# giuliop/AlgoPlonk

Hardware: AMD Instinct MI355X
Metric: proofs/sec (higher is better)
Workload: dtype u32x8 (Montgomery Fr/Fp)

## Files before the change

### algoplonk_amd/_lib.py

```python
from __future__ import annotations

import ctypes as C
import os

_HERE = os.path.dirname(os.path.abspath(__file__))
LIB_PATH = os.environ.get("APK_LIB") or os.path.join(_HERE, "libapk.so")

APK_BN254 = 0
APK_BLS12_381 = 1
APK_OK = 0
APK_ERR_ARG, APK_ERR_HIP, APK_ERR_STATE, APK_ERR_WITNESS, APK_ERR_VERIFY = 1, 2, 3, 4, 5
ABI_VERSION = 5
G1_MAX = 96
G2_MAX = 192
MAX_COMMITMENTS = 2
NB_BLINDING = 9

SYMBOLS = [
    "apk_last_error", "apk_abi_version", "apk_device_count", "apk_g1_bytes", "apk_fp_bytes",
    "apk_ctx_create", "apk_ctx_destroy", "apk_msm_ctx_create", "apk_ctx_get_vk", "apk_msm_g1", "apk_msm_g1_device", "apk_msm_g1_batch_device", "apk_ctx_set_commit_hook", "apk_device_copy", "apk_ntt",
    "apk_prove", "apk_prove_device", "apk_verify", "apk_verify_ex", "apk_g2_decompress", "apk_g2_mul_generator", "apk_g1_mul_batch", "apk_g1_decompress", "apk_g1_to_lagrange", "apk_marshal_proof", "apk_marshal_public_inputs",
    "apk_fe_from_be", "apk_fe_to_be", "apk_hash_fr", "apk_host_fe_op", "apk_host_g1_op", "apk_g1_sum",
    "apk_device_fe_op", "apk_device_g1_op", "apk_host_feu_op", "apk_device_feu_op", "apk_feu_shape", "apk_device_poly_op",
    "apk_device_alloc", "apk_device_free", "apk_device_upload", "apk_device_download",
    "apk_host_alloc", "apk_host_free", "apk_host_register", "apk_host_unregister",
    "apk_stats_enable", "apk_stats_read", "apk_paths_read",
    "apk_ctx_set_wire_hook", "apk_coset_ntt_device",
    "apk_comm_create", "apk_comm_destroy", "apk_comm_rank", "apk_comm_world", "apk_comm_barrier", "apk_comm_max_f64", "apk_comm_bind",
    "apk_comm_transport", "apk_msm_g1_sharded", "apk_comm_split_begin", "apk_comm_split_end", "apk_comm_serve", "apk_comm_set_compute",
    "apk_comm_commit", "apk_comm_wires", "apk_comm_rccl_ranks", "apk_comm_rccl_selftest",
    "apk_comm_commit_local", "apk_comm_spmd_begin", "apk_comm_spmd_end", "apk_comm_allgather_device", "apk_comm_subcoset_active",
    "apk_ctx_set_subcoset", "apk_comm_transport_reason", "apk_comm_link_probe", "apk_comm_phase_ms", "apk_ctx_msm_window",
    "apk_verify_batch", "apk_g1_lincomb_segments", "apk_device_sched_read", "apk_runtime_read",
    "apk_kzg_open", "apk_kzg_open_device", "apk_kzg_batch_open", "apk_kzg_batch_open_device", "apk_kzg_verify", "apk_kzg_batch_verify",
    "apk_kzg_fold_challenge", "apk_kzg_shape",
    "apk_kzg_open_lagrange", "apk_kzg_open_lagrange_device", "apk_kzg_batch_open_lagrange", "apk_kzg_batch_open_lagrange_device",
    "apk_kzg_lagrange_shape",
    "apk_kzg_open_multi", "apk_kzg_open_multi_device", "apk_kzg_batch_verify_multi", "apk_kzg_multi_weights",
    "apk_kzg_open_multi_lagrange", "apk_kzg_open_multi_lagrange_device",
    "apk_kzg_all_prepare", "apk_kzg_open_all", "apk_kzg_open_all_device",
    "apk_kzg_cosets_prepare", "apk_kzg_open_cosets", "apk_kzg_open_cosets_device", "apk_kzg_verify_coset",
    "apk_kzg_batch_verify_cosets", "apk_kzg_cosets_weights", "apk_kzg_cosets_fold", "apk_kzg_cosets_phase_ms",
    "apk_proof_blob_len", "apk_unmarshal_proof", "apk_unmarshal_public_inputs", "apk_verify_blob", "apk_verify_batch_keys", "apk_verify_blobs",
]


class ApkError(RuntimeError):
    def __init__(self, code: int, msg: str):
        super().__init__("libapk error %d: %s" % (code, msg))
        self.code = code


class CircuitDesc(C.Structure):
    _fields_ = [
        ("curve", C.c_int), ("device", C.c_int), ("n", C.c_uint64), ("nb_public", C.c_uint32),
        ("nb_commitments", C.c_uint32), ("srs_g1", C.c_void_p), ("srs_g1_lagrange", C.c_void_p),
        ("ql", C.c_void_p), ("qr", C.c_void_p), ("qm", C.c_void_p), ("qo", C.c_void_p), ("qk", C.c_void_p),
        ("perm", C.c_void_p), ("qcp", C.c_void_p * MAX_COMMITMENTS),
        ("commitment_constraint_index", C.c_uint32 * MAX_COMMITMENTS), ("msm_window", C.c_int), ("slots", C.c_int),
    ]


class Vk(C.Structure):
    _fields_ = [
        ("ql", C.c_uint8 * G1_MAX), ("qr", C.c_uint8 * G1_MAX), ("qm", C.c_uint8 * G1_MAX), ("qo", C.c_uint8 * G1_MAX),
        ("qk", C.c_uint8 * G1_MAX), ("s", (C.c_uint8 * G1_MAX) * 3), ("qcp", (C.c_uint8 * G1_MAX) * MAX_COMMITMENTS),
        ("size_inv", C.c_uint8 * 32), ("generator", C.c_uint8 * 32), ("coset_shift", C.c_uint8 * 32),
    ]


class Proof(C.Structure):
    _fields_ = [
        ("curve", C.c_uint32), ("nb_commitments", C.c_uint32),
        ("lro", (C.c_uint8 * G1_MAX) * 3), ("z", C.c_uint8 * G1_MAX), ("h", (C.c_uint8 * G1_MAX) * 3),
        ("bsb22", (C.c_uint8 * G1_MAX) * MAX_COMMITMENTS), ("batched_h", C.c_uint8 * G1_MAX),
        ("claimed_values", (C.c_uint8 * 32) * (6 + MAX_COMMITMENTS)), ("zshift_h", C.c_uint8 * G1_MAX),
        ("zshift_value", C.c_uint8 * 32),
        ("gamma", C.c_uint8 * 32), ("beta", C.c_uint8 * 32), ("alpha", C.c_uint8 * 32), ("zeta", C.c_uint8 * 32),
        ("gamma_kzg", C.c_uint8 * 32),
    ]


class VerifyingKey(C.Structure):
    _fields_ = [
        ("curve", C.c_int), ("n", C.c_uint64), ("nb_public", C.c_uint32), ("nb_commitments", C.c_uint32),
        ("ql", C.c_uint8 * G1_MAX), ("qr", C.c_uint8 * G1_MAX), ("qm", C.c_uint8 * G1_MAX), ("qo", C.c_uint8 * G1_MAX),
        ("qk", C.c_uint8 * G1_MAX), ("s", (C.c_uint8 * G1_MAX) * 3), ("qcp", (C.c_uint8 * G1_MAX) * MAX_COMMITMENTS),
        ("commitment_constraint_index", C.c_uint32 * MAX_COMMITMENTS), ("g1", C.c_uint8 * G1_MAX),
        ("g2", (C.c_uint8 * G2_MAX) * 2),
    ]


class VerifyTrace(C.Structure):
    _fields_ = [
        ("gamma", C.c_uint8 * 32), ("beta", C.c_uint8 * 32), ("alpha", C.c_uint8 * 32), ("zeta", C.c_uint8 * 32),
        ("pi", C.c_uint8 * 32), ("lin_at_zeta", C.c_uint8 * 32), ("gamma_kzg", C.c_uint8 * 32), ("folded_claim", C.c_uint8 * 32),
        ("lin_commitment", C.c_uint8 * G1_MAX), ("folded_digest", C.c_uint8 * G1_MAX),
    ]


class VerifyBatchTrace(C.Structure):
    _fields_ = [
        ("d", C.c_uint8 * 32), ("rho", (C.c_uint8 * 32) * 4), ("lin_commitment", (C.c_uint8 * G1_MAX) * 4),
        ("a", C.c_uint8 * G1_MAX), ("b", C.c_uint8 * G1_MAX), ("folds", C.c_uint32),
    ]


class VerifyKeysTrace(C.Structure):
    _fields_ = [
        ("d", C.c_uint8 * 32), ("rho", (C.c_uint8 * 32) * 4), ("lin_commitment", (C.c_uint8 * G1_MAX) * 4),
        ("a", C.c_uint8 * G1_MAX), ("b", C.c_uint8 * G1_MAX), ("groups", C.c_uint32), ("folds", C.c_uint32),
    ]


class KzgVk(C.Structure):
    _fields_ = [("curve", C.c_int), ("g1", C.c_uint8 * G1_MAX), ("g2", (C.c_uint8 * G2_MAX) * 2)]


class Stats(C.Structure):
    _fields_ = [
        ("msm_accumulate_ms", C.c_double), ("msm_accumulate_launches", C.c_uint64), ("msm_pairs", C.c_uint64),
        ("msm_total_ms", C.c_double), ("msm_batches", C.c_uint64), ("ntt_ms", C.c_double), ("ntt_elements", C.c_uint64),
        ("prove_ms", C.c_double), ("proofs", C.c_uint64), ("round_ms", C.c_double * 4), ("host_lincomb_ms", C.c_double),
        ("msm_sort_ms", C.c_double), ("msm_tail_ms", C.c_double),
    ]


class PathCounts(C.Structure):
    _names = ["proofs", "msm_batches", "msm_sort_two_level", "msm_sort_two_level_by_load", "msm_sort_fused", "msm_lean_tail",
              "msm_rowcol_serial", "msm_combine_quad", "msm_small_units", "msm_one_launch", "msm_lagrange_wires", "ntt_sequences",
              "ntt_radix4", "ntt_radix4_by_load", "tail_fill_proofs", "host_lincomb_pooled", "msm_units_by_load", "host_inputs",
              "gang_proofs", "gang_msm_launches", "gang_ntt_launches", "gang_kernel_launches", "forms_by_device_load"]
    _later = ["msm_inplace"]
    _fields_ = [(n, C.c_uint64) for n in _names + _later]

    def as_dict(self) -> dict:
        return {n: int(getattr(self, n)) for n in self._names + self._later}


class DeviceSched(C.Structure):
    _names = ["contexts", "max_streams", "streams_in_use", "streams_peak", "proofs_in_flight", "proofs_peak", "waiting", "device_wide"]
    _fields_ = [(n, C.c_uint32) for n in _names]

    def as_dict(self) -> dict:
        return {n: int(getattr(self, n)) for n in self._names}


HWQ_UNSET, HWQ_UNREADABLE = -1, -2


class Runtime(C.Structure):
    _names = ["hw_queues_found", "hw_queues_left", "hw_queues_need", "hw_queues_written", "hw_queues_now", "first_hip_call",
              "hw_queues_at_first_hip", "reserved"]
    _fields_ = [(n, C.c_int32) for n in _names]

    def as_dict(self) -> dict:
        return {n: int(getattr(self, n)) for n in self._names if n != "reserved"}


POLY_VECS, POLY_FRS, POLY_INTS, POLY_OUTS = 32, 24, 8, 6
(POLY_GRAND_PRODUCT, POLY_SCAN, POLY_QUOTIENT, POLY_MERGE, POLY_EVAL, POLY_LINCOMB, POLY_DERIVE_POWERS, POLY_KZG_QUOTIENT, POLY_BLIND,
 POLY_BLIND3, POLY_TAIL, POLY_KZG_QUOTIENT2) = range(12)


class PolyArgs(C.Structure):
    _fields_ = [("vec", C.c_void_p * POLY_VECS), ("len", C.c_uint64 * POLY_VECS), ("fr", (C.c_uint8 * 32) * POLY_FRS),
                ("iv", C.c_int64 * POLY_INTS), ("out", C.c_void_p * POLY_OUTS), ("out_len", C.c_uint64 * POLY_OUTS)]


COMMIT_HOOK = C.CFUNCTYPE(C.c_int, C.c_void_p, C.c_int, C.c_uint32, C.POINTER(C.c_void_p), C.POINTER(C.c_uint32), C.c_void_p)


WIRE_HOOK = C.CFUNCTYPE(C.c_int, C.c_void_p, C.c_uint32, C.POINTER(C.c_void_p), C.POINTER(C.c_uint32), C.POINTER(C.c_void_p))

CP_MSM = C.CFUNCTYPE(C.c_int, C.c_void_p, C.c_int, C.c_uint32, C.POINTER(C.c_void_p), C.POINTER(C.c_uint64), C.POINTER(C.c_uint64), C.c_void_p)
CP_COSET = C.CFUNCTYPE(C.c_int, C.c_void_p, C.c_void_p, C.c_uint64, C.c_void_p)
CP_ALLOC = C.CFUNCTYPE(C.c_int, C.c_void_p, C.c_size_t, C.POINTER(C.c_void_p))
CP_RELEASE = C.CFUNCTYPE(C.c_int, C.c_void_p, C.c_void_p)
CP_COPY = C.CFUNCTYPE(C.c_int, C.c_void_p, C.c_void_p, C.c_void_p, C.c_size_t, C.c_int)


class Compute(C.Structure):
    _fields_ = [("user", C.c_void_p), ("msm_batch", CP_MSM), ("coset_ntt", CP_COSET), ("alloc", CP_ALLOC), ("release", CP_RELEASE),
                ("copy", CP_COPY), ("g1_bytes", C.c_size_t), ("n", C.c_uint64)]


def _load() -> C.CDLL:
    if not os.path.exists(LIB_PATH):
        raise ImportError(
            "libapk.so not found at %s - build it with `make -C algoplonk_amd/csrc` "
            "(there is no CPU fallback for the HIP path)" % LIB_PATH)
    lib = C.CDLL(LIB_PATH)
    vp, u64, i32, sz = C.c_void_p, C.c_uint64, C.c_int, C.c_size_t
    lib.apk_last_error.restype = C.c_char_p
    lib.apk_abi_version.restype = i32
    lib.apk_device_count.argtypes = [C.POINTER(i32)]
    lib.apk_g1_bytes.argtypes = [i32]; lib.apk_g1_bytes.restype = sz
    lib.apk_fp_bytes.argtypes = [i32]; lib.apk_fp_bytes.restype = sz
    lib.apk_ctx_create.argtypes = [C.POINTER(CircuitDesc), C.POINTER(vp)]
    lib.apk_ctx_destroy.argtypes = [vp]; lib.apk_ctx_destroy.restype = None
    lib.apk_msm_ctx_create.argtypes = [i32, i32, vp, u64, i32, C.POINTER(vp)]
    lib.apk_ctx_get_vk.argtypes = [vp, C.POINTER(Vk)]
    lib.apk_msm_g1.argtypes = [vp, i32, vp, u64, vp]
    lib.apk_msm_g1_device.argtypes = [vp, i32, vp, u64, vp]
    lib.apk_msm_g1_batch_device.argtypes = [vp, i32, C.c_uint32, vp, vp, vp, vp]
    lib.apk_ctx_set_commit_hook.argtypes = [vp, COMMIT_HOOK, vp]
    lib.apk_device_copy.argtypes = [vp, vp, vp, sz]
    lib.apk_ntt.argtypes = [vp, i32, i32, i32, vp]
    lib.apk_prove.argtypes = [vp, vp, vp, vp, vp, vp, vp, C.POINTER(Proof)]
    lib.apk_prove_device.argtypes = [vp, vp, vp, vp, vp, vp, vp, C.POINTER(Proof)]
    lib.apk_verify.argtypes = [C.POINTER(VerifyingKey), C.POINTER(Proof), vp]
    lib.apk_verify_ex.argtypes = [C.POINTER(VerifyingKey), C.POINTER(Proof), vp, C.c_uint32, C.POINTER(VerifyTrace)]
    lib.apk_verify_batch.argtypes = [i32, C.POINTER(VerifyingKey), C.POINTER(Proof), C.POINTER(vp), C.POINTER(C.c_uint32), C.c_uint32,
                                     C.POINTER(i32), C.POINTER(VerifyBatchTrace)]
    if hasattr(lib, "apk_verify_batch_keys"):
        lib.apk_verify_batch_keys.argtypes = [i32, C.POINTER(VerifyingKey), C.c_uint32, C.POINTER(C.c_uint32), C.POINTER(Proof), C.POINTER(vp),
                                              C.POINTER(C.c_uint32), C.c_uint32, C.POINTER(i32), C.POINTER(VerifyKeysTrace)]
        lib.apk_proof_blob_len.argtypes = [i32, C.c_uint32]; lib.apk_proof_blob_len.restype = sz
        lib.apk_unmarshal_proof.argtypes = [i32, vp, sz, C.POINTER(Proof)]
        lib.apk_unmarshal_public_inputs.argtypes = [i32, vp, sz, vp, C.c_uint32, C.POINTER(C.c_uint32)]
        lib.apk_verify_blob.argtypes = [C.POINTER(VerifyingKey), vp, sz, vp, sz, C.POINTER(VerifyTrace)]
        lib.apk_verify_blobs.argtypes = [i32, C.POINTER(VerifyingKey), C.c_uint32, C.POINTER(C.c_uint32), C.POINTER(vp), C.POINTER(sz),
                                         C.POINTER(vp), C.POINTER(sz), C.c_uint32, C.POINTER(i32), C.POINTER(VerifyKeysTrace)]
    lib.apk_g1_lincomb_segments.argtypes = [i32, i32, vp, vp, C.POINTER(u64), C.c_uint32, vp]
    lib.apk_g2_decompress.argtypes = [i32, vp, vp]
    lib.apk_g2_mul_generator.argtypes = [i32, vp, vp]
    lib.apk_g1_mul_batch.argtypes = [i32, i32, vp, vp, u64, vp]
    lib.apk_g1_decompress.argtypes = [i32, i32, vp, u64, vp]
    lib.apk_g1_to_lagrange.argtypes = [i32, i32, vp, u64, vp]
    lib.apk_marshal_proof.argtypes = [C.POINTER(Proof), vp, sz, C.POINTER(sz)]
    lib.apk_marshal_public_inputs.argtypes = [i32, vp, C.c_uint32, vp, sz]
    lib.apk_fe_from_be.argtypes = [i32, i32, vp, vp]
    lib.apk_fe_to_be.argtypes = [i32, i32, vp, vp]
    lib.apk_hash_fr.argtypes = [i32, vp, vp]
    lib.apk_host_fe_op.argtypes = [i32, i32, i32, vp, vp, vp]
    lib.apk_host_g1_op.argtypes = [i32, i32, vp, vp, vp]
    lib.apk_device_fe_op.argtypes = [i32, i32, i32, i32, u64, vp, vp, vp]
    lib.apk_device_g1_op.argtypes = [i32, i32, i32, u64, vp, vp, vp]
    lib.apk_host_feu_op.argtypes = [i32, i32, i32, u64, vp, vp]
    lib.apk_device_feu_op.argtypes = [i32, i32, i32, i32, u64, vp, vp]
    lib.apk_feu_shape.argtypes = [i32, i32, C.POINTER(i32), C.POINTER(i32), C.POINTER(C.c_uint32)]
    if hasattr(lib, "apk_device_poly_op"):
        lib.apk_device_poly_op.argtypes = [i32, i32, i32, C.POINTER(PolyArgs)]
    lib.apk_g1_sum.argtypes = [i32, vp, u64, vp]
    lib.apk_device_alloc.argtypes = [vp, sz, C.POINTER(vp)]
    lib.apk_device_free.argtypes = [vp, vp]
    lib.apk_device_upload.argtypes = [vp, vp, vp, sz]
    lib.apk_device_download.argtypes = [vp, vp, vp, sz]
    lib.apk_host_alloc.argtypes = [i32, sz, C.POINTER(vp)]
    lib.apk_host_free.argtypes = [vp]
    lib.apk_host_register.argtypes = [vp, sz]
    lib.apk_host_unregister.argtypes = [vp]
    lib.apk_stats_enable.argtypes = [vp, i32]
    lib.apk_stats_read.argtypes = [vp, C.POINTER(Stats), i32]
    lib.apk_paths_read.argtypes = [vp, C.POINTER(PathCounts), i32]
    if hasattr(lib, "apk_device_sched_read"):
        lib.apk_device_sched_read.argtypes = [i32, C.POINTER(DeviceSched), i32]
    if hasattr(lib, "apk_runtime_read"):
        lib.apk_runtime_read.argtypes = [C.POINTER(Runtime)]
    lib.apk_ctx_msm_window.argtypes = [vp]
    lib.apk_ctx_set_wire_hook.argtypes = [vp, WIRE_HOOK, vp]
    lib.apk_coset_ntt_device.argtypes = [vp, vp, u64, vp]
    lib.apk_comm_create.argtypes = [i32, i32, C.c_char_p, i32, C.POINTER(vp)]
    lib.apk_comm_destroy.argtypes = [vp]; lib.apk_comm_destroy.restype = None
    lib.apk_comm_rank.argtypes = [vp]
    lib.apk_comm_world.argtypes = [vp]
    lib.apk_comm_barrier.argtypes = [vp]
    lib.apk_comm_max_f64.argtypes = [vp, C.POINTER(C.c_double)]
    lib.apk_comm_bind.argtypes = [vp, vp]
    lib.apk_comm_transport.argtypes = [vp]; lib.apk_comm_transport.restype = C.c_char_p
    lib.apk_comm_rccl_ranks.argtypes = [vp]
    lib.apk_comm_transport_reason.argtypes = [vp]; lib.apk_comm_transport_reason.restype = C.c_char_p
    lib.apk_comm_link_probe.argtypes = [vp, sz, sz, C.POINTER(C.c_double), C.POINTER(C.c_double)]
    lib.apk_comm_phase_ms.argtypes = [vp, C.POINTER(C.c_double), i32]
    lib.apk_comm_rccl_selftest.argtypes = [i32, C.POINTER(i32)]
    lib.apk_msm_g1_sharded.argtypes = [vp, vp, u64, vp]
    lib.apk_comm_split_begin.argtypes = [vp]
    lib.apk_comm_split_end.argtypes = [vp]
    lib.apk_comm_serve.argtypes = [vp, C.POINTER(u64)]
    lib.apk_comm_set_compute.argtypes = [vp, C.POINTER(Compute)]
    lib.apk_comm_commit.argtypes = [vp, i32, C.c_uint32, vp, vp, vp]
    lib.apk_comm_wires.argtypes = [vp, C.c_uint32, vp, vp, vp]
    lib.apk_comm_commit_local.argtypes = [vp, i32, C.c_uint32, vp, vp, vp]
    lib.apk_comm_spmd_begin.argtypes = [vp]
    lib.apk_comm_spmd_end.argtypes = [vp]
    lib.apk_comm_allgather_device.argtypes = [vp, vp, C.c_size_t]
    lib.apk_comm_subcoset_active.argtypes = [vp]
    lib.apk_ctx_set_subcoset.argtypes = [vp, i32, i32, vp, vp]
    lib.apk_kzg_open.argtypes = [vp, vp, u64, vp, vp, vp]
    lib.apk_kzg_open_device.argtypes = [vp, vp, u64, vp, vp, vp]
    lib.apk_kzg_batch_open.argtypes = [vp, C.c_uint32, vp, vp, vp, vp, vp, sz, vp, vp, vp]
    lib.apk_kzg_batch_open_device.argtypes = [vp, C.c_uint32, vp, vp, vp, vp, vp, sz, vp, vp, vp]
    lib.apk_kzg_verify.argtypes = [C.POINTER(KzgVk), vp, vp, vp, vp]
    lib.apk_kzg_batch_verify.argtypes = [C.POINTER(KzgVk), C.c_uint32, vp, vp, vp, vp, sz, vp]
    lib.apk_kzg_fold_challenge.argtypes = [i32, C.c_uint32, vp, vp, vp, vp, sz, vp]
    lib.apk_kzg_shape.argtypes = [C.POINTER(i32), C.POINTER(i32)]
    if hasattr(lib, "apk_kzg_open_lagrange"):
        lib.apk_kzg_open_lagrange.argtypes = [vp, vp, u64, vp, vp, vp]
        lib.apk_kzg_open_lagrange_device.argtypes = [vp, vp, u64, vp, vp, vp]
        lib.apk_kzg_batch_open_lagrange.argtypes = [vp, C.c_uint32, vp, vp, vp, vp, sz, vp, vp, vp]
        lib.apk_kzg_batch_open_lagrange_device.argtypes = [vp, C.c_uint32, vp, vp, vp, vp, sz, vp, vp, vp]
        lib.apk_kzg_lagrange_shape.argtypes = [C.POINTER(i32), C.POINTER(i32)]
    if hasattr(lib, "apk_kzg_open_multi"):
        lib.apk_kzg_open_multi.argtypes = [vp, C.c_uint32, vp, vp, vp, vp, vp]
        lib.apk_kzg_open_multi_device.argtypes = [vp, C.c_uint32, vp, vp, vp, vp, vp]
        lib.apk_kzg_batch_verify_multi.argtypes = [C.POINTER(KzgVk), i32, C.c_uint32, vp, vp, vp, vp]
        lib.apk_kzg_multi_weights.argtypes = [C.POINTER(KzgVk), C.c_uint32, vp, vp, vp, vp, vp]
    if hasattr(lib, "apk_kzg_open_multi_lagrange"):
        lib.apk_kzg_open_multi_lagrange.argtypes = [vp, C.c_uint32, vp, vp, vp, vp]
        lib.apk_kzg_open_multi_lagrange_device.argtypes = [vp, C.c_uint32, vp, vp, vp, vp]
    if hasattr(lib, "apk_kzg_open_all"):
        lib.apk_kzg_all_prepare.argtypes = [vp, vp, u64]
        lib.apk_kzg_open_all.argtypes = [vp, vp, u64, vp, vp]
        lib.apk_kzg_open_all_device.argtypes = [vp, vp, u64, vp, vp]
    if hasattr(lib, "apk_kzg_open_cosets"):
        lib.apk_kzg_cosets_prepare.argtypes = [vp, vp, u64, C.c_uint32]
        lib.apk_kzg_open_cosets.argtypes = [vp, vp, u64, vp, vp]
        lib.apk_kzg_open_cosets_device.argtypes = [vp, vp, u64, vp, vp]
        lib.apk_kzg_verify_coset.argtypes = [C.POINTER(KzgVk), vp, vp, u64, C.c_uint32, u64, vp, vp, vp]
    if hasattr(lib, "apk_kzg_batch_verify_cosets"):
        u32 = C.c_uint32
        lib.apk_kzg_batch_verify_cosets.argtypes = [C.POINTER(KzgVk), i32, vp, vp, u64, u32, u32, vp, u32, C.POINTER(u32), C.POINTER(u64), vp, vp]
        lib.apk_kzg_cosets_weights.argtypes = [C.POINTER(KzgVk), vp, u64, u32, u32, vp, u32, C.POINTER(u32), C.POINTER(u64), vp, vp, vp]
        lib.apk_kzg_cosets_fold.argtypes = [i32, i32, u64, u32, u32, C.POINTER(u64), vp, vp, vp]
        lib.apk_kzg_cosets_phase_ms.argtypes = [C.POINTER(C.c_double)]
    return lib


lib = _load()


def check(code: int) -> None:
    if code != APK_OK:
        raise ApkError(code, (lib.apk_last_error() or b"").decode())


def device_sched(device: int = 0, reset: bool = False) -> dict:
    if not hasattr(lib, "apk_device_sched_read"):
# ... 19 lines not shown
```

### algoplonk_amd/csrc/apk_api.cpp

```cpp
#include <stdarg.h>
#include <stdio.h>
#include <stdlib.h>
#include <string.h>
#include <atomic>
#include <mutex>
#include <string>
#include <type_traits>

#include <hip/hip_runtime_api.h>

#include "backend.h"
#include "device_sched.h"
#include "ec.h"
#include "kernels_kzg.h"
#include "kernels_kzg_lagrange.h"
#include "plonk_protocol.h"
#include "poly_run.h"
#include "proof_codec.h"
#include "runtime_env.h"
#include "selftest_ops.h"

namespace apk {

static thread_local std::string g_err;
// ... 442 lines not shown
}
int apk_ctx_set_commit_hook(apk_ctx* ctx, apk_commit_hook hook, void* user) { NEED_CTX(); return ctx->be->set_commit_hook(hook, user); }
int apk_device_copy(apk_ctx* ctx, void* d, const void* s, size_t b) { NEED_CTX(); return ctx->be->dev_copy(d, s, b); }
int apk_ctx_set_wire_hook(apk_ctx* ctx, apk_wire_hook hook, void* user) { NEED_CTX(); return ctx->be->set_wire_hook(hook, user); }
int apk_ctx_set_subcoset(apk_ctx* ctx, int k, int world, apk_gather_hook hook, void* user) { NEED_CTX(); return ctx->be->set_subcoset(k, world, hook, user); }
int apk_coset_ntt_device(apk_ctx* ctx, const void* d_in, uint64_t len, void* d_out) { NEED_CTX(); return ctx->be->coset_ntt_dev(d_in, len, d_out); }
int apk_ntt(apk_ctx* ctx, int which, int inverse, int coset, void* data) {
    NEED_CTX(); if (!data) { set_error("null data"); return APK_ERR_ARG; }
    return ctx->be->ntt(which, inverse, coset, data);
}
int apk_prove(apk_ctx* ctx, const void* L, const void* R, const void* O, const void* pub, const void* bl,
              const void* const* pi2, apk_proof* out) {
    NEED_CTX();
    return ctx->be->prove(L, R, O, false, pub, bl, pi2, out);
}
int apk_prove_device(apk_ctx* ctx, const void* L, const void* R, const void* O, const void* pub, const void* bl,
                     const void* const* pi2, apk_proof* out) {
    NEED_CTX();
    return ctx->be->prove(L, R, O, true, pub, bl, pi2, out);
}
static int host_mem_device(int device) {
    int ndev = 0;
    runtime_checkpoint();
    hipError_t e = hipGetDeviceCount(&ndev);
    if (e != hipSuccess || ndev == 0) { (void)hipGetLastError(); set_error("no HIP device available (%s); libapk has no CPU fallback", e == hipSuccess ? "0 devices" : hipGetErrorString(e)); return APK_ERR_HIP; }
    if (device < 0 || device >= ndev) { set_error("device %d out of range (%d devices)", device, ndev); return APK_ERR_ARG; }
    e = hipSetDevice(device);
    if (e != hipSuccess) { set_error("hipSetDevice: %s", hipGetErrorString(e)); return APK_ERR_HIP; }
    return APK_OK;
}
int apk_host_alloc(int device, size_t bytes, void** p) {
    if (!p || bytes == 0) { set_error("null argument"); return APK_ERR_ARG; }
    *p = nullptr;
    int rc = host_mem_device(device);
    if (rc != APK_OK) return rc;
    hipError_t e = hipHostMalloc(p, bytes, hipHostMallocPortable);
    if (e != hipSuccess) { (void)hipGetLastError(); *p = nullptr; set_error("hipHostMalloc(%zu): %s", bytes, hipGetErrorString(e)); return APK_ERR_HIP; }
    return APK_OK;
}
int apk_host_free(void* p) {
    if (!p) return APK_OK;
    hipError_t e = hipHostFree(p);
    if (e != hipSuccess) { (void)hipGetLastError(); set_error("hipHostFree: %s", hipGetErrorString(e)); return APK_ERR_HIP; }
    return APK_OK;
}
int apk_host_register(void* p, size_t bytes) {
    if (!p || bytes == 0) { set_error("null argument"); return APK_ERR_ARG; }
    int rc = host_mem_device(0);
    if (rc != APK_OK) return rc;
    hipError_t e = hipHostRegister(p, bytes, hipHostRegisterPortable);
    if (e != hipSuccess) { (void)hipGetLastError(); set_error("hipHostRegister(%zu): %s", bytes, hipGetErrorString(e)); return APK_ERR_HIP; }
    return APK_OK;
}
int apk_host_unregister(void* p) {
    if (!p) return APK_OK;
    hipError_t e = hipHostUnregister(p);
    if (e != hipSuccess) { (void)hipGetLastError(); set_error("hipHostUnregister: %s", hipGetErrorString(e)); return APK_ERR_HIP; }
    return APK_OK;
}

int apk_device_alloc(apk_ctx* ctx, size_t bytes, void** p) { NEED_CTX(); return ctx->be->dev_alloc(bytes, p); }
int apk_device_free(apk_ctx* ctx, void* p) { NEED_CTX(); return ctx->be->dev_free(p); }
int apk_device_upload(apk_ctx* ctx, void* d, const void* s, size_t b) { NEED_CTX(); return ctx->be->dev_upload(d, s, b); }
int apk_device_download(apk_ctx* ctx, void* d, const void* s, size_t b) { NEED_CTX(); return ctx->be->dev_download(d, s, b); }
int apk_stats_enable(apk_ctx* ctx, int en) { NEED_CTX(); return ctx->be->stats_enable(en); }
int apk_stats_read(apk_ctx* ctx, apk_stats* out, int reset) { NEED_CTX(); if (!out) { set_error("null out"); return APK_ERR_ARG; } return ctx->be->stats_read(out, reset); }
int apk_ctx_msm_window(apk_ctx* ctx) { if (!ctx || !ctx->be) return 0; return ctx->be->msm_window(); }
int apk_device_sched_read(int device, apk_device_sched* out, int reset) {
    if (!out) { set_error("null out"); return APK_ERR_ARG; }
    if (device < 0 || device >= 4096) { set_error("device %d out of range", device); return APK_ERR_ARG; }
    memset(out, 0, sizeof *out);
    out->max_streams = (uint32_t)sched_max_streams();
    out->device_wide = sched_device_wide() ? 1u : 0u;
    DeviceSched* sc = device_sched_for(device);
    if (!sc) return APK_OK;
    const DeviceSched::Counts c = sc->read(reset != 0);
    out->contexts = c.contexts; out->max_streams = c.max_streams;
    out->streams_in_use = c.streams_in_use; out->streams_peak = c.streams_peak;
    out->proofs_in_flight = c.proofs_in_flight; out->proofs_peak = c.proofs_peak;
    out->waiting = c.waiting;
    return APK_OK;
}
int apk_paths_read(apk_ctx* ctx, apk_path_counts* out, int reset) { NEED_CTX(); if (!out) { set_error("null out"); return APK_ERR_ARG; } return ctx->be->paths_read(out, reset); }
int apk_runtime_read(apk_runtime* out) {
    if (!out) { set_error("null out"); return APK_ERR_ARG; }
    memset(out, 0, sizeof *out);
    out->hw_queues_found = g_runtime.found; out->hw_queues_left = g_runtime.left;
    out->hw_queues_need = g_runtime.need; out->hw_queues_written = g_runtime.written;
    out->hw_queues_now = hwq_parse(getenv("GPU_MAX_HW_QUEUES"));
    out->first_hip_call = g_runtime.first_hip.load();
    out->hw_queues_at_first_hip = g_runtime.at_first_hip.load();
    return APK_OK;
}

int apk_g1_mul_batch(int curve, int device, const void* base, const void* scalars, uint64_t count, void* out) {
    if (!base || !scalars || !out) { set_error("null argument"); return APK_ERR_ARG; }
    if (count == 0) return APK_OK;
    if (count >= (1ull << 31)) { set_error("count too large"); return APK_ERR_ARG; }
    runtime_checkpoint();
    if (curve == APK_BN254) return g1_mul_batch_bn254(device, base, scalars, count, out);
    if (curve == APK_BLS12_381) return g1_mul_batch_bls12381(device, base, scalars, count, out);
    set_error("unsupported curve: %d", curve);
    return APK_ERR_ARG;
}

int apk_g1_decompress(int curve, int device, const uint8_t* compressed, uint64_t count, void* out) {
    if (!compressed || !out) { set_error("null argument"); return APK_ERR_ARG; }
    if (count == 0) return APK_OK;
    if (count >= (1ull << 31)) { set_error("count too large"); return APK_ERR_ARG; }
    runtime_checkpoint();
    if (curve == APK_BN254) return g1_decompress_bn254(device, compressed, count, out);
    if (curve == APK_BLS12_381) return g1_decompress_bls12381(device, compressed, count, out);
    set_error("unsupported curve: %d", curve);
    return APK_ERR_ARG;
}

int apk_g1_to_lagrange(int curve, int device, const void* points, uint64_t n, void* out) {
    if (!points || !out) { set_error("null argument"); return APK_ERR_ARG; }
    runtime_checkpoint();
    if (curve == APK_BN254) return g1_to_lagrange_bn254(device, points, n, out);
    if (curve == APK_BLS12_381) return g1_to_lagrange_bls12381(device, points, n, out);
    set_error("unsupported curve: %d", curve);
    return APK_ERR_ARG;
}

int apk_host_fe_op(int curve, int field, int op, const void* a, const void* b, void* out) {
    if (!a || !out) { set_error("null argument"); return APK_ERR_ARG; }
    if (curve == APK_BN254) return selftest_status(field ? fe_op_t<FpBN254>(op, a, b, out) : fe_op_t<FrBN254>(op, a, b, out), "field", op);
    if (curve == APK_BLS12_381) return selftest_status(field ? fe_op_t<FpBLS12381>(op, a, b, out) : fe_op_t<FrBLS12381>(op, a, b, out), "field", op);
    set_error("unsupported curve: %d", curve);
    return APK_ERR_ARG;
}

int apk_host_g1_op(int curve, int op, const void* p, const void* q, void* out) {
    if (!p || !out || (op != 2 && !q)) { set_error("null argument"); return APK_ERR_ARG; }
    if (curve == APK_BN254) return selftest_status(g1_op_t<FrBN254, FpBN254>(op, p, q, out), "g1", op);
    if (curve == APK_BLS12_381) return selftest_status(g1_op_t<FrBLS12381, FpBLS12381>(op, p, q, out), "g1", op);
    set_error("unsupported curve: %d", curve);
    return APK_ERR_ARG;
}

int apk_feu_shape(int curve, int field, int* ul, int* ub, uint32_t* headroom) {
    if (!ul || !ub || !headroom) { set_error("null argument"); return APK_ERR_ARG; }
    if (curve == APK_BN254) { field ? feu_shape_t<FpBN254>(ul, ub, headroom) : feu_shape_t<FrBN254>(ul, ub, headroom); return APK_OK; }
    if (curve == APK_BLS12_381) { field ? feu_shape_t<FpBLS12381>(ul, ub, headroom) : feu_shape_t<FrBLS12381>(ul, ub, headroom); return APK_OK; }
    set_error("unsupported curve: %d", curve);
    return APK_ERR_ARG;
}

int apk_host_feu_op(int curve, int field, int op, uint64_t count, const void* in, void* out) {
    if (count && (!in || !out)) { set_error("null argument"); return APK_ERR_ARG; }
    const uint32_t* i = static_cast<const uint32_t*>(in);
    uint32_t* o = static_cast<uint32_t*>(out);
    if (curve == APK_BN254) return field ? host_feu_batch<FpBN254>(op, count, i, o) : host_feu_batch<FrBN254>(op, count, i, o);
    if (curve == APK_BLS12_381) return field ? host_feu_batch<FpBLS12381>(op, count, i, o) : host_feu_batch<FrBLS12381>(op, count, i, o);
    set_error("unsupported curve: %d", curve);
    return APK_ERR_ARG;
}

int apk_device_fe_op(int curve, int field, int op, int device, uint64_t count, const void* a, const void* b, void* out) {
    if (count && (!a || !b || !out)) { set_error("null argument"); return APK_ERR_ARG; }
    if (!seam_args(curve, count, (op >= 0 && op <= 4) || (op >= 10 && op <= 14), op, "field")) return APK_ERR_ARG;
    if (count == 0) return APK_OK;
    runtime_checkpoint();
    return curve == APK_BN254 ? fe_op_device_bn254(device, field, op, count, a, b, out) : fe_op_device_bls12381(device, field, op, count, a, b, out);
}

int apk_device_feu_op(int curve, int field, int op, int device, uint64_t count, const void* in, void* out) {
    if (count && (!in || !out)) { set_error("null argument"); return APK_ERR_ARG; }
    if (!seam_args(curve, count, (op >= 0 && op <= 29) || (op >= 40 && op <= 48), op, "unsaturated")) return APK_ERR_ARG;
    if (count == 0) return APK_OK;
    runtime_checkpoint();
    return curve == APK_BN254 ? feu_op_device_bn254(device, field, op, count, in, out) : feu_op_device_bls12381(device, field, op, count, in, out);
}

int apk_device_g1_op(int curve, int op, int device, uint64_t count, const void* p, const void* q, void* out) {
    const bool unary = op == 2 || op == 21;
    if (count && (!p || !out || (!unary && !q))) { set_error("null argument"); return APK_ERR_ARG; }
    if (!seam_args(curve, count, (op >= 0 && op <= 3) || (op >= 10 && op <= 15) || op == 20 || op == 21, op, "g1")) return APK_ERR_ARG;
    if (count == 0) return APK_OK;
    runtime_checkpoint();
    return curve == APK_BN254 ? g1_op_device_bn254(device, op, count, p, q, out) : g1_op_device_bls12381(device, op, count, p, q, out);
}

int apk_device_poly_op(int curve, int op, int device, const apk_poly_args* args) {
    if (curve != APK_BN254 && curve != APK_BLS12_381) { set_error("unsupported curve: %d", curve); return APK_ERR_ARG; }
    if (const char* why = poly_op_check(op, args)) { set_error("polynomial-stage op %d: %s", op, why); return APK_ERR_ARG; }
    runtime_checkpoint();
    return curve == APK_BN254 ? poly_op_device_bn254(device, op, args) : poly_op_device_bls12381(device, op, args);
}

int apk_g1_sum(int curve, const void* points, uint64_t count, void* out) {
    if (!out || (count && !points)) { set_error("null argument"); return APK_ERR_ARG; }
    if (curve == APK_BN254) return g1_sum_t<FpBN254>(points, count, out);
    if (curve == APK_BLS12_381) return g1_sum_t<FpBLS12381>(points, count, out);
    set_error("unsupported curve: %d", curve);
    return APK_ERR_ARG;
}

int apk_fe_from_be(int curve, int field, const uint8_t* be, void* out) {
    if (!be || !out) { set_error("null argument"); return APK_ERR_ARG; }
    return host_fe_from_be(curve, field, be, out);
}
int apk_fe_to_be(int curve, int field, const void* in, uint8_t* be) {
    if (!be || !in) { set_error("null argument"); return APK_ERR_ARG; }
    return host_fe_to_be(curve, field, in, be);
}

int apk_marshal_proof(const apk_proof* p, uint8_t* out, size_t cap, size_t* len) {
    if (!p || !out || !len) { set_error("null argument"); return APK_ERR_ARG; }
    CodecError err;
    const int rc = marshal_proof(p, out, cap, len, &err);
    if (rc != APK_OK) set_error("%s", err.msg);
    return rc;
}

int apk_marshal_public_inputs(int curve, const void* pub, uint32_t nb_public, uint8_t* out, size_t cap) {
    if ((!pub && nb_public) || !out) { set_error("null argument"); return APK_ERR_ARG; }
    CodecError err;
    const int rc = marshal_public_inputs(curve, pub, nb_public, out, cap, &err);
    if (rc != APK_OK) set_error("%s", err.msg);
    return rc;
}

int apk_hash_fr(int curve, const void* g1_affine, void* out_fr) {
    if (!g1_affine || !out_fr) { set_error("null argument"); return APK_ERR_ARG; }
    if (!apk_g1_bytes(curve)) { set_error("unsupported curve: %d", curve); return APK_ERR_ARG; }
    auto hash = [&](auto proto) {
        using Proto = decltype(proto);
        typename Proto::Aff p;
        memcpy(&p, g1_affine, sizeof p);
        const typename Proto::Fr r = Proto::hash_fr(p);
        memcpy(out_fr, &r, sizeof r);
    };
    if (curve == APK_BN254) hash(PlonkProtocol<FrBN254, FpBN254>{}); else hash(PlonkProtocol<FrBLS12381, FpBLS12381>{});
    return APK_OK;
}

}
```

### algoplonk_amd/csrc/backend.h

```cpp
#pragma once
#include <stdint.h>
#include <stddef.h>
#include <stdarg.h>
#include <stdio.h>
#include "../../include/apk.h"

namespace apk {

void set_error(const char* fmt, ...);

int env_int(const char* name, int dflt, int lo, int hi);

bool ctx_alive(const void* ctx);

class DeviceSched;
DeviceSched* device_sched_for(int device);
int device_stream_pool(int device, void** streams, int cap, int* count);

struct Backend {
    virtual ~Backend() {}
    virtual int init(const apk_circuit_desc* d) = 0;
    virtual int init_msm_only(int device, const void* bases, uint64_t count, int msm_window) = 0;
    virtual int get_vk(apk_vk* out) = 0;
    virtual int msm(int basis, const void* scalars, uint64_t len, bool on_device, void* out) = 0;
    virtual int msm_batch(int basis, uint32_t count, const void* const* d_scalars, const uint64_t* offsets, const uint64_t* lens, void* out) = 0;
    virtual int kzg_open(const void* poly, uint64_t len, bool on_device, const void* point, void* out_h, void* out_value) = 0;
    virtual int kzg_batch_open(uint32_t count, const void* const* polys, const uint64_t* lens, bool on_device, const void* digests,
                               const void* point, const uint8_t* extra, size_t extra_len, void* out_h, void* out_values, void* out_gamma) = 0;
    virtual int kzg_open_multi(uint32_t count, const void* const* polys, const uint64_t* lens, bool on_device, const void* points,
                               void* out_h, void* out_values) = 0;
    virtual int kzg_open_lagrange(const void* evals, uint64_t len, bool on_device, const void* point, void* out_h, void* out_value) = 0;
    virtual int kzg_batch_open_lagrange(uint32_t count, const void* const* evals, bool on_device, const void* digests, const void* point,
                                        const uint8_t* extra, size_t extra_len, void* out_h, void* out_values, void* out_gamma) = 0;
    virtual int kzg_open_multi_lagrange(uint32_t count, const void* const* evals, bool on_device, const void* points, void* out_h,
                                        void* out_values) = 0;
    virtual int kzg_all_prepare(const void* srs_g1, uint64_t count) = 0;
    virtual int kzg_open_all(const void* poly, uint64_t len, bool on_device, void* out_h, void* out_values) = 0;
    virtual int kzg_cosets_prepare(const void* srs_g1, uint64_t count, uint32_t coset_size) = 0;
    virtual int kzg_open_cosets(const void* poly, uint64_t len, bool on_device, void* out_h, void* out_values) = 0;
    virtual int set_commit_hook(apk_commit_hook fn, void* user) = 0;
    virtual int dev_copy(void* d, const void* s, size_t bytes) = 0;
    virtual int set_wire_hook(apk_wire_hook fn, void* user) = 0;
    virtual int set_subcoset(int k, int G, apk_gather_hook fn, void* user) = 0;
    virtual int device_ordinal() = 0;
    virtual int msm_window() = 0;
    virtual uint64_t domain_size() = 0;
    virtual int coset_ntt_dev(const void* d_in, uint64_t len, void* d_out) = 0;
    virtual int ntt(int which, int inverse, int coset, void* data) = 0;
    virtual int prove(const void* L, const void* R, const void* O, bool on_device, const void* pub, const void* blinding,
                      const void* const* pi2, apk_proof* out) = 0;
    virtual int dev_alloc(size_t bytes, void** p) = 0;
    virtual int dev_free(void* p) = 0;
    virtual int dev_upload(void* d, const void* s, size_t bytes) = 0;
    virtual int dev_download(void* d, const void* s, size_t bytes) = 0;
    virtual int stats_enable(int enable) = 0;
    virtual int stats_read(apk_stats* out, int reset) = 0;
    virtual int paths_read(apk_path_counts* out, int reset) = 0;
};

int g1_mul_batch_bn254(int device, const void* base, const void* scalars, uint64_t count, void* out);
int g1_mul_batch_bls12381(int device, const void* base, const void* scalars, uint64_t count, void* out);
int g1_decompress_bn254(int device, const uint8_t* in, uint64_t count, void* out);
int g1_decompress_bls12381(int device, const uint8_t* in, uint64_t count, void* out);
int g1_to_lagrange_bn254(int device, const void* points, uint64_t n, void* out);
int g1_to_lagrange_bls12381(int device, const void* points, uint64_t n, void* out);
int fe_op_device_bn254(int device, int field, int op, uint64_t count, const void* a, const void* b, void* out);
int fe_op_device_bls12381(int device, int field, int op, uint64_t count, const void* a, const void* b, void* out);
int feu_op_device_bn254(int device, int field, int op, uint64_t count, const void* in, void* out);
int feu_op_device_bls12381(int device, int field, int op, uint64_t count, const void* in, void* out);
int g1_op_device_bn254(int device, int op, uint64_t count, const void* p, const void* q, void* out);
int g1_op_device_bls12381(int device, int op, uint64_t count, const void* p, const void* q, void* out);
int poly_op_device_bn254(int device, int op, const apk_poly_args* args);
int poly_op_device_bls12381(int device, int op, const apk_poly_args* args);
int g1_lincomb_segments_bn254(int device, const void* points, const void* scalars, const uint64_t* seg, uint32_t nb_segments, void* out);
int g1_lincomb_segments_bls12381(int device, const void* points, const void* scalars, const uint64_t* seg, uint32_t nb_segments, void* out);
int g1_check_points_bn254(int device, const void* points, uint64_t count, uint8_t* flags);
int g1_check_points_bls12381(int device, const void* points, uint64_t count, uint8_t* flags);
int kzg_cosets_fold_bn254(int device, int log_l, uint32_t count, const void* values, const void* scale, const void* step, const void* tw, void* out);
int kzg_cosets_fold_bls12381(int device, int log_l, uint32_t count, const void* values, const void* scale, const void* step, const void* tw, void* out);
Backend* make_backend_bn254();
Backend* make_backend_bls12381();

int host_fe_from_be(int curve, int field, const uint8_t* be, void* out);
int host_fe_to_be(int curve, int field, const void* in, uint8_t* be);

}
```

### algoplonk_amd/csrc/backend_impl.h

```cpp
#pragma once
#include <hip/hip_runtime.h>
#include <algorithm>
#include <atomic>
#include <chrono>
#include <condition_variable>
#include <memory>
#include <new>
#include <mutex>
#include <string.h>
#include <time.h>
#include <vector>

#include "backend.h"
#include "dev_buf.h"
#include "slot_pinned.h"
#include "msm_run.h"
#include "kzg_run.h"
#include "kzg_all_run.h"
#include "kzg_cosets_run.h"
#include "ntt_run.h"
#include "kernels_poly.h"
#include "poly_run.h"
#include "gang_run.h"
#include "setup_run.h"
#include "host_msm.h"
#include "slot_gate.h"
#include "gang.h"
#include "plonk_protocol.h"

namespace apk {

template <class FRP, class FPP, int CURVE_ID>
class CurveBackend : public Backend {
  public:
    using Fr = Fe<FRP>;
    using Fp = Fe<FPP>;
    using Aff = Affine<FPP>;
    using Pt = XYZZ<FPP>;
    using PtU = XYZZ<FPP, FeU<FPP>>;
    using Proto = PlonkProtocol<FRP, FPP>;

    static Fr fr_u64(uint64_t v) {
        Fr a = Fr::zero();
        a.l[0] = (uint32_t)v;
        a.l[1] = (uint32_t)(v >> 32);
        return Fr::to_mont(a);
    }

    static_assert(PIN_AFF + MSM_MAX_BATCH * sizeof(Aff) <= PIN_XYZZ, "a proof's batch of affine commitments fits its region");
    static_assert(PIN_XYZZ + MSM_ARGS_MAX * sizeof(Pt) <= PIN_FR, "the XYZZ sums of a launch sequence fit their region");
    static_assert(PIN_FR + (EVAL_MAX > KZG_MAX_POLYS ? EVAL_MAX : KZG_MAX_POLYS) * sizeof(Fr) <= PIN_TAIL, "evaluations and an opening's values fit the scalar region");

    struct ProverKnobs {
        int lc_threads = env_int("APK_HOST_LINCOMB_THREADS", FPP::N <= 8 ? 1 : 3, 1, 8);
        bool host_glv = env_int("APK_HOST_GLV", 1, 0, 1) != 0;
        bool host_fixed = env_int("APK_HOST_FIXED", 1, 0, 1) != 0;
        int powers_derive = env_int("APK_POWERS_DERIVE", 1, 0, 1);
        int open_pair = env_int("APK_OPEN_PAIR", 1, 0, 1);
        int lin_early_h = env_int("APK_LIN_EARLY_H", 1, 0, 1);
        int tail_fill = env_int("APK_TAIL_FILL", 1, 0, 2);
    };
    static const ProverKnobs& prover_knobs() { static const ProverKnobs k{}; return k; }

    struct GraphKey {
        const void* table; MsmBatchArgs a;
        bool operator==(const GraphKey& o) const { return table == o.table && memcmp(&a, &o.a, sizeof a) == 0; }
    };
    struct Slot {
        hipStream_t stream = nullptr;
        hipStream_t own_stream = nullptr;
        Slot* lead = nullptr;
        int gang_idx = 0;
        bool in_gang = false;
        uint32_t res_off = 0;
        uint32_t res_write_off = 0;
        Gang gang;
        GangRecorder cmds;
        hipEvent_t ev0 = nullptr, ev1 = nullptr, ev2 = nullptr, ev3 = nullptr;
        size_t index = 0;
        DevBuf wl, wr, wo;
        DevBuf cl, cr, co, cz;
        DevBuf qk_lag, qk_can;
        DevBuf ratio, zlag, scan_tot;
        DevBuf el, er, eo, ez, eqk;
        DevBuf quot, hcan;
        DevBuf pw_z, pw_zi, pw_zw, pw_zwi;
        DevBuf tmp2, folded, tmp, q1, q2;
        DevBuf eval_partial, eval_result;
        DevBuf pi2_can[APK_MAX_COMMITMENTS], epi2[APK_MAX_COMMITMENTS];
        DevBuf scratch_in;
        KzgScratch<FRP> kzg;
        KzgAllScratch<FRP, FPP> kzg_all;
        KzgCosetsScratch<FRP, FPP> kzg_cosets;
        DevBuf ntt_wide;
        MsmWorkspace<FPP> msm;
        void* h_pinned = nullptr;
        uint32_t pending_pts = 0;
        uint8_t* d_pinned = nullptr;
        std::vector<std::pair<GraphKey, hipGraphExec_t>> graphs;
        bool hook_pending = false;
        int hook_basis = 0;
        MsmBatchArgs hook_args{};
        DevBuf sc_gather;
        DevBuf tail_flag;
        uint32_t epoch = 0;
        hipStream_t side = nullptr;
        hipEvent_t ev_acc = nullptr, ev_side = nullptr;
        hipEvent_t ev_sync = nullptr;
        int mark_acc = 0; bool side_pending = false;
    };

    int curve_ = CURVE_ID;
    int device_ = 0;
    uint32_t n_ = 0, log_n_ = 0, n4_ = 0;
    uint32_t nb_public_ = 0, nb_commit_ = 0;
    uint32_t cci_[APK_MAX_COMMITMENTS] = {0, 0};
    MsmCtxPlan msm_ctx_{};
    bool msm_only_ = false;
    std::unique_ptr<HostPool> lc_pool_;
    bool many_slots_ = false;
    int gang_cap_ = 1;
    uint32_t ws_batch_ = MSM_MAX_BATCH;
    Gang::Launcher gang_launcher_;
    uint32_t msm_bases_ = 0;
    Fr omega_, omega_inv_, omega4_, omega4_inv_, shift_, shift_inv_, n_inv_, n4_inv_;
    Fr zh_inv_[4];
    DevBuf tw_n_, twu_n_, twi_n_, tw_4n_, twi_4n_, coset_pre_, coset_post_inv_, scales_;
    DevBuf twu_n_x_, twi_n_x_, tw_4n_x_, twi_4n_x_;
    bool ntt_twu_ = false;
    DevBuf x4_, l0_4_;
    DevBuf s_lag_[3], ql_c_, qr_c_, qm_c_, qo_c_, qk_c_, s_c_[3], qcp_c_[APK_MAX_COMMITMENTS];
    DevBuf qk_lag_trace_;
    bool qk_direct_ = false;
    DevBuf eqk_trace_, inj_tab_[QK_INJECT_MAX];
    std::vector<uint32_t> inj_row_;
    std::vector<Fr> inj_trace_val_;
    DevBuf eql_, eqr_, eqm_, eqo_, es_[3], eqcp_[APK_MAX_COMMITMENTS];
    MsmTables tab_can_, tab_lag_;
    int wires_lag_mode_ = -1;
    DevBuf srs_keep_;
    Aff lag_dk_[3];
    std::mutex lag_mu_;
    std::atomic<bool> lag_ready_{false};
    std::atomic<bool> lag_failed_{false};
    std::atomic<uint32_t> wire_density_pm_{0xffffffffu};
    std::atomic<uint32_t> proof_seq_{0};
    enum { VK_QL, VK_QR, VK_QM, VK_QO, VK_QK, VK_S1, VK_S2, VK_S3, VK_QCP };
    Aff vk_pts_[8 + APK_MAX_COMMITMENTS];
    HostFixedBase<FPP> vk_fixed_;
    KzgAllTables<FRP, FPP> all_tab_;
    std::mutex all_mu_;
    std::atomic<bool> all_ready_{false};
    bool tw_ready_ = false;
    KzgCosetsTables cos_tab_;
    std::atomic<uint32_t> cos_l_{0};
    std::vector<Slot*> slots_;
    std::vector<hipStream_t> stream_pool_;
    bool owns_streams_ = false;
    SlotGate gate_;
    struct InputSet {
        DevBuf w[3], pi2[APK_MAX_COMMITMENTS];
        hipStream_t copy = nullptr;
        hipEvent_t ready = nullptr;
        size_t index = 0;
    };
    std::vector<InputSet*> in_sets_;
    SlotGate in_gate_;
    hipStream_t copy_stream_ = nullptr;
    std::mutex mu_;
    apk_commit_hook hook_ = nullptr;
    void* hook_user_ = nullptr;
    apk_wire_hook wire_hook_ = nullptr;
    void* wire_hook_user_ = nullptr;
    struct SubCoset {
        int k = 0, G = 1, glog = 0;
        apk_gather_hook hook = nullptr;
        void* user = nullptr;
        DevBuf pre[2], post;
        Fr rho_inv[8];
        bool on() const { return G > 1 && hook; }
    } sc_;
    enum PathIdx { P_PROOFS, P_MSM_BATCHES, P_SORT2, P_SORT2_LOAD, P_SORT_FUSED, P_LEAN_TAIL, P_ROWCOL_SERIAL, P_COMBINE_QUAD, P_SMALL_UNITS,
                   P_ONE_LAUNCH, P_LAGRANGE_WIRES, P_NTT_SEQ, P_NTT_R4, P_NTT_R4_LOAD, P_TAIL_FILL, P_LINCOMB_POOL, P_UNIT_LOADED, P_HOST_INPUTS, P_GANG_PROOFS, P_GANG_MSM, P_GANG_NTT, P_GANG_KERNELS, P_DEVICE_LOAD, P_MSM_INPLACE, P_COUNT };
    std::atomic<uint64_t> paths_[P_COUNT] = {};
    void path(PathIdx i) { paths_[i].fetch_add(1, std::memory_order_relaxed); }
    bool device_load_over(int thr, bool* foreign = nullptr) {
        int own = 0;
        const int dev = gate_.load(&own);
        if (foreign) *foreign = dev > thr && own <= thr;
        return dev > thr;
    }
    int paths_read(apk_path_counts* out, int reset) override {
        static_assert(sizeof(apk_path_counts) >= P_COUNT * sizeof(uint64_t), "apk_path_counts holds every counter");
        memset(out, 0, sizeof *out);
        uint64_t* o = reinterpret_cast<uint64_t*>(out);
        for (int i = 0; i < P_COUNT; i++) o[i] = reset ? paths_[i].exchange(0, std::memory_order_relaxed) : paths_[i].load(std::memory_order_relaxed);
        return APK_OK;
    }
    bool stats_on_ = false;
    uint32_t simds_ = 1024;
    std::mutex stats_mu_;
    apk_stats stats_{};

    ~CurveBackend() override {
        (void)hipSetDevice(device_);
        gate_.detach();
        for (hipStream_t st : stream_pool_) if (st) (void)hipStreamSynchronize(st);
        if (copy_stream_) (void)hipStreamSynchronize(copy_stream_);
        for (InputSet* is : in_sets_) {
            if (is->ready) (void)hipEventDestroy(is->ready);
            delete is;
        }
        if (copy_stream_) (void)hipStreamDestroy(copy_stream_);
        for (Slot* s : slots_) {
            for (auto& e : s->graphs) (void)hipGraphExecDestroy(e.second);
            if (s->ev0) (void)hipEventDestroy(s->ev0);
            if (s->ev1) (void)hipEventDestroy(s->ev1);
            if (s->ev2) (void)hipEventDestroy(s->ev2);
            if (s->ev3) (void)hipEventDestroy(s->ev3);
            if (s->h_pinned) (void)hipHostFree(s->h_pinned);
            if (s->side) { (void)hipStreamSynchronize(s->side); (void)hipStreamDestroy(s->side); }
            if (s->ev_acc) (void)hipEventDestroy(s->ev_acc);
            if (s->ev_side) (void)hipEventDestroy(s->ev_side);
            if (s->ev_sync) (void)hipEventDestroy(s->ev_sync);
            delete s;
        }
        if (owns_streams_) for (hipStream_t st : stream_pool_) if (st) (void)hipStreamDestroy(st);
    }

    int run_ntt_batch(hipStream_t st, int which, bool inverse, int count, const Fr* const* ins, Fr* const* outs, const uint32_t* in_lens,
                      uint32_t out_len, const Fr* pre, const Fr* post, const Fr* scale, int sub_log = 0, bool semi = false) {
        Slot* m = gang_member();
        if (m && m->in_gang && st == m->stream && count <= NTT_MAX_BATCH) {
            NttReq<Fr> nr{};
            nr.which = which; nr.inverse = inverse; nr.count = count;
            for (int i = 0; i < count; i++) { nr.ins[i] = ins[i]; nr.outs[i] = outs[i]; nr.in_lens[i] = in_lens[i]; }
            nr.out_len = out_len; nr.pre = pre; nr.post = post; nr.scale = scale; nr.sub_log = sub_log; nr.semi = semi;
            GangReq r;
            r.kind = GANG_KIND_NTT; r.args = &nr; r.member = m;
            const int rc = m->lead->gang.meet(m->gang_idx, r, gang_launcher_);
            if (rc != APK_OK) set_error("%s", r.err.c_str());
            return rc;
        }
        return run_ntt_batch_now(st, which, inverse, count, ins, outs, in_lens, out_len, pre, post, scale, sub_log, semi);
    }
    const Fr* ntt_table(int which, bool inverse) const {
        if (ntt_twu_) return which ? (inverse ? ptr<Fr>(twi_4n_x_) : ptr<Fr>(tw_4n_x_)) : (inverse ? ptr<Fr>(twi_n_x_) : ptr<Fr>(twu_n_x_));
        return which ? (inverse ? ptr<Fr>(twi_4n_) : ptr<Fr>(tw_4n_)) : (inverse ? ptr<Fr>(twi_n_) : ptr<Fr>(twu_n_));
    }
    int run_ntt_batch_now(hipStream_t st, int which, bool inverse, int count, const Fr* const* ins, Fr* const* outs, const uint32_t* in_lens,
                          uint32_t out_len, const Fr* pre, const Fr* post, const Fr* scale, int sub_log = 0, bool semi = false) {
        const int log_n = (which ? (int)log_n_ + 2 : (int)log_n_) - sub_log;
        Slot* owner = nullptr;
        for (Slot* s : slots_) if (s->own_stream == st || (s->side && s->side == st)) owner = s;
        bool busy_now = false, busy_foreign = false;
        if (slots_.size() > 2 && ntt_plan_reads_load(log_n)) busy_now = device_load_over(1, &busy_foreign);
        const NttPlanIn in{log_n, count, out_len, sub_log, semi, (uint32_t)sizeof(FeU<FRP>), owner != nullptr, busy_now, busy_foreign};
        const NttPlan plan = ntt_plan(ntt_knobs(), in);
        if (plan.rc != APK_OK) { set_error("%s", plan.message); return plan.rc; }
        NttBatch nb{};
        for (int i = 0; i < count; i++) { nb.in[i] = ins[i]; nb.out[i] = outs[i]; nb.in_len[i] = in_lens[i]; }
        if (plan.needs_wide) for (int i = 0; i < count; i++) nb.wide[i] = ptr<FeU<FRP>>(owner->ntt_wide) + ((size_t)i << log_n);
        static constexpr PathIdx PATH_OF_BIT[] = {P_NTT_SEQ, P_NTT_R4, P_NTT_R4_LOAD, P_DEVICE_LOAD};
        for (uint32_t i = 0; i < sizeof PATH_OF_BIT / sizeof PATH_OF_BIT[0]; i++) if (plan.paths >> i & 1u) path(PATH_OF_BIT[i]);
        Slot* timed = stats_on_ ? owner : nullptr;
        if (timed) HIPCHK(hipEventRecord(timed->ev2, st));
        CHK(ntt_launch<FRP>(st, plan, nb, count, ntt_table(which, inverse), ntt_twu_, pre, post, scale));
        if (timed) {
// ... 85 lines not shown
        HIPCHK(hipGraphLaunch(exec, s.stream));
        s.pending_pts = a.batch;
        return APK_OK;
    }

    int run_msm_body(Slot& s, const MsmTables& T, const MsmBatchArgs& a) {
        hipStream_t st = s.stream;
        MsmBatchIn in{};
        in.batch = a.batch; in.len = a.len; in.offset = a.offset;
        in.n_bases = T.n_bases; in.ctx_bases = msm_bases_;
        in.simds = simds_; in.slots = (uint32_t)slots_.size();
        if (slots_.size() > 2) in.others_busy = device_load_over(1, &in.others_foreign);
        in.scan_runs = APK_PHASE(32);
        in.ws_batch = ws_batch_;
        in.lt_max = MsmQuad<FPP>::LT;
        in.counts_words = s.msm.counts.bytes / 4; in.sort_tmp_bytes = s.msm.sort_tmp.bytes;
        in.has_sort_tmp = s.msm.sort_tmp.p != nullptr; in.has_ptot2 = s.msm.ptot2.p != nullptr;
        const MsmBatchPlan p = msm_plan_batch(msm_ctx_, msm_knobs(), in);
        static constexpr PathIdx PATH_OF_BIT[] = {P_UNIT_LOADED, P_SMALL_UNITS, P_SORT2, P_SORT2_LOAD, P_SORT_FUSED, P_LEAN_TAIL, P_COMBINE_QUAD, P_ROWCOL_SERIAL, P_DEVICE_LOAD, P_MSM_INPLACE};
        for (uint32_t i = 0; i < sizeof PATH_OF_BIT / sizeof PATH_OF_BIT[0]; i++) if (p.paths >> i & 1u) path(PATH_OF_BIT[i]);
        if (p.rc == APK_ERR_ARG) { set_error("%s", p.message); return p.rc; }
        if (p.rc == APK_OK) {
            path(P_MSM_BATCHES);
            if (s.res_write_off + a.batch > (uint32_t)MSM_ARGS_MAX) { set_error("msm: result area overflow"); return APK_ERR_STATE; }
        }
        Pt* const res_out = s.d_pinned ? pin_dev<Pt>(s.d_pinned, PIN_XYZZ) + s.res_write_off : ptr<Pt>(s.msm.result_xyzz);
        MsmEvents ev;
        if (stats_on_) { ev.before = s.ev0; ev.scanned = s.ev2; ev.accumulated = s.ev3; ev.reduced = s.ev1; }
        ev.acc = s.ev_acc; ev.mark_acc = s.mark_acc;
        CHK((msm_launch_batch<FRP, FPP>(st, msm_ctx_, s.msm, ptr<Aff>(T.table), T.n_bases, a, p, res_out, ev)));
        if (!s.d_pinned) HIPCHK(hipMemcpyAsync(pin_host<Pt>(s.h_pinned, PIN_XYZZ) + s.res_write_off, s.msm.result_xyzz.p, a.batch * sizeof(Pt), hipMemcpyDeviceToHost, st));
        s.pending_pts = a.batch;
        if (stats_on_) {
            HIPCHK(hipEventSynchronize(s.ev1));
            float tot = 0, acc = 0, srt = 0, tail = 0;
            HIPCHK(hipEventElapsedTime(&tot, s.ev0, s.ev1));
            HIPCHK(hipEventElapsedTime(&acc, s.ev2, s.ev3));
            HIPCHK(hipEventElapsedTime(&srt, s.ev0, s.ev2));
            HIPCHK(hipEventElapsedTime(&tail, s.ev3, s.ev1));
            std::lock_guard<std::mutex> g(stats_mu_);
            stats_.msm_sort_ms += srt;
            stats_.msm_tail_ms += tail;
            stats_.msm_total_ms += tot;
            stats_.msm_batches += 1;
            stats_.msm_accumulate_ms += acc;
            stats_.msm_accumulate_launches += 1;
            for (uint32_t b = 0; b < a.batch; b++) stats_.msm_pairs += a.len[b];
        }
        return APK_OK;
    }

    static Slot*& hook_slot() { static thread_local Slot* p = nullptr; return p; }

    int commit(Slot& s, const MsmTables& T, int basis, const MsmBatchArgs& a) {
        if (!hook_ && s.in_gang) {
            MsmReq mr{&T, a};
            GangReq r;
            r.kind = GANG_KIND_MSM; r.args = &mr; r.member = &s;
            const int rc = s.lead->gang.meet(s.gang_idx, r, gang_launcher_);
            if (rc != APK_OK) set_error("%s", r.err.c_str());
            return rc;
        }
        if (!hook_) return run_msm(s, T, a);
        for (uint32_t b = 0; b < a.batch; b++)
            if (a.len[b] > T.n_bases || a.offset[b] > T.n_bases - a.len[b]) { set_error("msm: %u scalars exceed the %u bases", a.len[b], T.n_bases); return APK_ERR_ARG; }
        s.hook_pending = true; s.hook_basis = basis; s.hook_args = a;
        s.hook_args.plain = T.plain ? 1u : 0u;
        return APK_OK;
    }

    int tail_fill(Slot& s) {
        const int on = prover_knobs().tail_fill;
        const int graphs = msm_knobs().graph;
        if (!on || graphs || hook_ || wire_hook_ || stats_on_ || !qk_direct_ || sc_.on()) return 0;
        if (gate_.load() != 1) return 0;
        if (!s.side) {
            int least = 0, greatest = 0;
            (void)hipDeviceGetStreamPriorityRange(&least, &greatest);
            if (hipStreamCreateWithPriority(&s.side, hipStreamNonBlocking, least) != hipSuccess) { s.side = nullptr; return 0; }
            if (hipEventCreateWithFlags(&s.ev_acc, hipEventDisableTiming) != hipSuccess ||
                hipEventCreateWithFlags(&s.ev_side, hipEventDisableTiming) != hipSuccess) return 0;
        }
        return s.ev_acc && s.ev_side ? on : 0;
    }
    int side_begin(Slot& s) { HIPCHK(hipStreamWaitEvent(s.side, s.ev_acc, 0)); return APK_OK; }
    int side_end(Slot& s) { HIPCHK(hipEventRecord(s.ev_side, s.side)); s.side_pending = true; return APK_OK; }

    int wait_stream(Slot& s) {
        static const int mode = env_int("APK_SYNC_BLOCKING", -1, -1, 2);
        static const int poll_us = env_int("APK_SYNC_POLL_US", 50, 1, 10000);
        const bool loaded = slots_.size() > 2 && device_load_over(2);
        if (s.ev_sync && (mode == 2 || (mode < 0 && loaded))) {
            HIPCHK(hipEventRecord(s.ev_sync, s.stream));
            for (;;) {
                const hipError_t e = hipEventQuery(s.ev_sync);
                if (e == hipSuccess) return APK_OK;
                if (e != hipErrorNotReady) { (void)hipGetLastError(); set_error("hipEventQuery: %s", hipGetErrorString(e)); return APK_ERR_HIP; }
                struct timespec ts = {0, (long)poll_us * 1000L};
                nanosleep(&ts, nullptr);
            }
        }
        if (mode == 1 && s.ev_sync) {
            HIPCHK(hipEventRecord(s.ev_sync, s.stream));
            HIPCHK(hipEventSynchronize(s.ev_sync));
            return APK_OK;
        }
        HIPCHK(hipStreamSynchronize(s.stream));
        return APK_OK;
    }

    int sync_results(Slot& s) {
        if (s.in_gang) {
            GangReq r;
            r.kind = GANG_KIND_FLUSH; r.member = &s;
            const int rc = s.lead->gang.meet(s.gang_idx, r, gang_launcher_);
            if (rc != APK_OK) { set_error("%s", r.err.c_str()); return rc; }
        }
        CHK(wait_stream(s));
        if (s.side_pending) { s.side_pending = false; HIPCHK(hipStreamWaitEvent(s.stream, s.ev_side, 0)); }
        if (s.hook_pending) {
            s.hook_pending = false;
            const MsmBatchArgs& a = s.hook_args;
            uint8_t pts[MSM_MAX_BATCH * sizeof(Aff)];
            hook_slot() = &s;
            const int rc = hook_(hook_user_, s.hook_basis, a.batch, a.scalars, a.len, pts);
            hook_slot() = nullptr;
            if (rc != APK_OK) { set_error("commit hook failed with %d", rc); return rc == APK_ERR_ARG ? APK_ERR_ARG : APK_ERR_STATE; }
            memcpy(pin_host<Aff>(s.h_pinned, PIN_AFF), pts, a.batch * sizeof(Aff));
            s.pending_pts = 0;
            return APK_OK;
        }
        const Slot& from = s.lead ? *s.lead : s;
        const Pt* g = pin_host<Pt>(from.h_pinned, PIN_XYZZ) + s.res_off;
        static_assert(MSM_MAX_BATCH <= HOST_AFFINE_BATCH, "a proof's batch of sums is one batch conversion");
        host_xyzz_batch_to_affine<FPP>(g, s.pending_pts, pin_host<Aff>(s.h_pinned, PIN_AFF));
        s.pending_pts = 0;
        return APK_OK;
    }

    int alloc_slot(Slot& s) {
        s.lead = &s;
        HIPCHK(hipEventCreate(&s.ev0));
        HIPCHK(hipEventCreate(&s.ev1));
        HIPCHK(hipEventCreate(&s.ev2));
        HIPCHK(hipEventCreate(&s.ev3));
        if (hipEventCreateWithFlags(&s.ev_sync, hipEventBlockingSync | hipEventDisableTiming) != hipSuccess) { (void)hipGetLastError(); s.ev_sync = nullptr; }
        HIPCHK(hipHostMalloc(&s.h_pinned, PIN_BYTES, hipHostMallocDefault));
        memset(s.h_pinned, 0, PIN_BYTES);
        static const int zero_copy = env_int("APK_ZERO_COPY", 1, 0, 1);
        if (zero_copy) {
            void* dp = nullptr;
            if (hipHostGetDevicePointer(&dp, s.h_pinned, 0) == hipSuccess) s.d_pinned = static_cast<uint8_t*>(dp);
            else (void)hipGetLastError();
        }
        const size_t fn = (size_t)n_ * sizeof(Fr), fn3 = (size_t)(n_ + 4) * sizeof(Fr), f4 = (size_t)n4_ * sizeof(Fr);
        if (msm_only_) {
            CHK(s.scratch_in.alloc((size_t)msm_bases_ * sizeof(Fr)));
            return s.msm.alloc(msm_ctx_, msm_knobs(), msm_bases_, 1, many_slots_);
        }
        CHK(s.wl.alloc(fn3)); CHK(s.wr.alloc(fn3)); CHK(s.wo.alloc(fn3));
        CHK(s.cl.alloc(fn3)); CHK(s.cr.alloc(fn3)); CHK(s.co.alloc(fn3)); CHK(s.cz.alloc(fn3));
        for (DevBuf* b : {&s.cl, &s.cr, &s.co, &s.cz}) HIPCHK(hipMemset(b->p, 0, fn3));
        CHK(s.qk_lag.alloc(fn)); CHK(s.qk_can.alloc(fn));
        CHK(s.ratio.alloc(fn)); CHK(s.zlag.alloc(fn));
        CHK(s.scan_tot.alloc((size_t)(2 * (cdiv(n_ + 4, SCAN_BLOCK) + 1) + 2) * sizeof(Fr)));
        CHK(s.el.alloc(f4)); CHK(s.er.alloc(f4)); CHK(s.eo.alloc(f4)); CHK(s.ez.alloc(f4)); CHK(s.eqk.alloc(f4));
// ... 881 lines not shown
        Slot* own = MaybeGuard::own(this);
        hipStream_t st = own ? own->stream : nullptr;
        HIPCHK(hipMemcpyAsync(dd, ss, bytes, hipMemcpyDeviceToDevice, st));
        HIPCHK(hipStreamSynchronize(st));
        return APK_OK;
    }

    int ntt(int which, int inverse, int coset, void* data) override {
        if (msm_only_) { set_error("MSM-only context has no NTT domain"); return APK_ERR_STATE; }
        HIPCHK(hipSetDevice(device_));
        SlotGuard g(this);
        Slot& s = *g.s;
        const uint32_t N = which ? n4_ : n_;
        if (coset && !which) { set_error("coset transforms are provided on the 4n domain"); return APK_ERR_ARG; }
        Fr* din = ptr<Fr>(s.scratch_in);
        Fr* dout = ptr<Fr>(s.quot);
        HIPCHK(hipMemcpyAsync(din, data, (size_t)N * sizeof(Fr), hipMemcpyHostToDevice, s.stream));
        if (coset == 2 && inverse) { set_error("the semi-canonical form exists for forward coset transforms only"); return APK_ERR_ARG; }
        if (!coset) {
            CHK(run_ntt(s.stream, which, inverse != 0, din, dout, N, N, nullptr, nullptr,
                        inverse ? ptr<Fr>(scales_) + (which ? 1 : 0) : nullptr));
        } else if (!inverse) {
            CHK(powers(s.stream, ptr<Fr>(s.hcan), N, shift_, fr_u64(32)));
            CHK(run_ntt(s.stream, 1, false, din, dout, N, N, ptr<Fr>(s.hcan), nullptr, nullptr, 0, coset == 2));
        } else {
            CHK(run_ntt(s.stream, 1, true, din, dout, N, N, nullptr, ptr<Fr>(coset_post_inv_), nullptr));
        }
        HIPCHK(hipMemcpyAsync(data, dout, (size_t)N * sizeof(Fr), hipMemcpyDeviceToHost, s.stream));
        HIPCHK(hipStreamSynchronize(s.stream));
        g.ok = true;
        return APK_OK;
    }

    int dev_alloc(size_t bytes, void** p) override { HIPCHK(hipSetDevice(device_)); HIPCHK(hipMalloc(p, bytes)); return APK_OK; }
    int dev_free(void* p) override { HIPCHK(hipSetDevice(device_)); HIPCHK(hipFree(p)); return APK_OK; }
    int dev_upload(void* dd, const void* s, size_t bytes) override { HIPCHK(hipSetDevice(device_)); HIPCHK(hipMemcpy(dd, s, bytes, hipMemcpyHostToDevice)); return APK_OK; }
    int dev_download(void* dd, const void* s, size_t bytes) override { HIPCHK(hipSetDevice(device_)); HIPCHK(hipMemcpy(dd, s, bytes, hipMemcpyDeviceToHost)); return APK_OK; }
    int stats_enable(int en) override { stats_on_ = en != 0; return APK_OK; }
    int stats_read(apk_stats* out, int reset) override {
        std::lock_guard<std::mutex> g(stats_mu_);
        *out = stats_;
        if (reset) stats_ = apk_stats{};
        return APK_OK;
    }

    int kzg_quotient(Slot& s, const Fr* f, uint32_t len, const Fr* pw, const Fr* pwi, bool z_is_zero, Fr* q) {
        return poly_kzg_quotient<FRP>(kl(), s.stream, f, len, pw, pwi, z_is_zero, ptr<Fr>(s.tmp), ptr<Fr>(s.scan_tot), q);
    }

    int eval_many(Slot& s, const EvalArgs<FRP>& ea, const Fr* pw, Fr* h_out) {
        hipStream_t st = s.stream;
        Fr* const twin = pin_dev_of(s.h_pinned, s.d_pinned, h_out, ea.count * sizeof(Fr));
        const bool direct = twin != nullptr;
        Fr* const ev_out = direct ? twin : ptr<Fr>(s.eval_result);
        CHK(poly_eval_many<FRP>(kl(), st, ea, pw, ptr<Fr>(s.eval_partial), ev_out));
        if (!direct) HIPCHK(hipMemcpyAsync(h_out, s.eval_result.p, ea.count * sizeof(Fr), hipMemcpyDeviceToHost, st));
        return APK_OK;
    }

    typename Proto::KeyPoints key_points() const {
        typename Proto::KeyPoints key{vk_pts_[VK_QL], vk_pts_[VK_QR], vk_pts_[VK_QM], vk_pts_[VK_QO], vk_pts_[VK_QK],
                                      vk_pts_[VK_S1], vk_pts_[VK_S2], vk_pts_[VK_S3], {}, nb_commit_};
        for (uint32_t k = 0; k < nb_commit_; k++) key.qcp[k] = vk_pts_[VK_QCP + k];
        return key;
    }

    static void store_pt(uint8_t* slot, const Aff& p) { memset(slot, 0, APK_G1_MAX_BYTES); memcpy(slot, &p, sizeof(Aff)); }

    struct ProofRun {
        Slot& s;
        InputSet* in;
        hipStream_t st;
        const Fr *dL, *dR, *dO;
        const Fr *pubv, *bl;
        const Fr* pi2[APK_MAX_COMMITMENTS];
        apk_proof* out;
        Aff bsb[APK_MAX_COMMITMENTS];
        Fr cval[APK_MAX_COMMITMENTS];
        Aff lro[3], zcom, hcom[3];
        Fr gamma, beta, beta_u, beta_u2, alpha, zeta, gk;
        uint8_t gamma_raw[32], beta_raw[32], alpha_raw[32], zeta_raw[32], gk_raw[32];
        typename Proto::KeyPoints key;
        int fill = 0;
        bool use_lag = false, measuring = false;
        std::chrono::steady_clock::time_point t_start, t_phase;
        double phase_ms[4] = {0, 0, 0, 0}, lincomb_ms = 0;
    };
    void mark(ProofRun& run, int r) {
        if (!stats_on_) return;
        const auto now = std::chrono::steady_clock::now();
        run.phase_ms[r] = std::chrono::duration<double, std::milli>(now - run.t_phase).count();
        run.t_phase = now;
    }
    struct LinTerm { const Fr* poly; uint32_t len; Aff com; Fr coef; };
    enum { LT_QL, LT_QR, LT_QM, LT_QO, LT_QK, LT_S3, LT_Z, LT_H1, LT_H2, LT_H3, LT_BSB, LT_MAX = LT_BSB + APK_MAX_COMMITMENTS };
    using HostSum = XYZZ<FPP, Fe64<FPP>>;

    int prove(const void* L, const void* R, const void* O, bool on_device, const void* pub, const void* blinding,
              const void* const* pi2, apk_proof* out) override;
    int round1_wires(ProofRun& run);
    int round2_grand_product(ProofRun& run);
    int round3_quotient(ProofRun& run);
    int round4_openings(ProofRun& run);
    int wire_route(ProofRun& run);
    uint32_t wire_route_finish(ProofRun& run);
    QuotientArgs<FRP> quotient_args(const ProofRun& run);
    int zeta_powers(ProofRun& run);
    Aff lin_commitment(ProofRun& run, const LinTerm* terms, int count, HostPool* pool, const HostSum* lin_h);
};

template <class FRP, class FPP, int CURVE_ID>
int CurveBackend<FRP, FPP, CURVE_ID>::setup_trace(const apk_circuit_desc* d) {
    Slot& s = *slots_[0];
    hipStream_t st = s.stream;
    const size_t fn = (size_t)n_ * sizeof(Fr), f4 = (size_t)n4_ * sizeof(Fr);
    {
        std::vector<Fr> l0(n_, n_inv_);
        HIPCHK(hipMemcpyAsync(s.tmp.p, l0.data(), fn, hipMemcpyHostToDevice, st));
        HIPCHK(hipStreamSynchronize(st));
        CHK(l0_4_.alloc(f4));
        CHK(coset_ntt_4n(st, ptr<Fr>(s.tmp), n_, ptr<Fr>(l0_4_)));
    }
    const void* cols[5] = {d->ql, d->qr, d->qm, d->qo, d->qk};
    DevBuf* can[5] = {&ql_c_, &qr_c_, &qm_c_, &qo_c_, &qk_c_};
    DevBuf* cos[4] = {&eql_, &eqr_, &eqm_, &eqo_};
    for (int i = 0; i < 5; i++) {
        CHK(can[i]->alloc(fn));
        HIPCHK(hipMemcpyAsync(s.wl.p, cols[i], fn, hipMemcpyHostToDevice, st));
        if (i == 4) { CHK(qk_lag_trace_.alloc(fn)); HIPCHK(hipMemcpyAsync(qk_lag_trace_.p, s.wl.p, fn, hipMemcpyDeviceToDevice, st)); }
        CHK(inv_ntt_n(st, ptr<Fr>(s.wl), ptr<Fr>(*can[i])));
        if (i < 4) {
            CHK(cos[i]->alloc(f4));
            CHK(coset_ntt_4n(st, ptr<Fr>(*can[i]), n_, ptr<Fr>(*cos[i])));
            scale_kernel<FRP><<<cdiv(n4_, POLY_THREADS), POLY_THREADS, 0, st>>>(ptr<Fr>(*cos[i]), fr_u64(i == 2 ? 1u << 10 : 1u << 5), n4_); KCHK();
        }
        HIPCHK(hipStreamSynchronize(st));
    }
    inj_row_.clear(); inj_trace_val_.clear();
    for (uint32_t i = 0; i < nb_public_; i++) inj_row_.push_back(i);
    for (uint32_t k = 0; k < nb_commit_; k++) inj_row_.push_back(nb_public_ + cci_[k]);
    qk_direct_ = inj_row_.size() <= (size_t)QK_INJECT_MAX && !getenv("APK_QK_NTT");
    if (qk_direct_) {
        CHK(eqk_trace_.alloc(f4));
        CHK(coset_ntt_4n(st, ptr<Fr>(qk_c_), n_, ptr<Fr>(eqk_trace_)));
        for (size_t j = 0; j < inj_row_.size(); j++) {
            const uint32_t row = inj_row_[j];
            if (row >= n_) { set_error("Qk row %u out of range", row); return APK_ERR_ARG; }
            inj_trace_val_.push_back(reinterpret_cast<const Fr*>(d->qk)[row]);
            if (row == 0) continue;
            CHK(inj_tab_[j].alloc(f4));
            CHK(powers(st, ptr<Fr>(s.tmp), n_, Fr::pow_u64(omega_inv_, row), n_inv_));
            CHK(coset_ntt_4n(st, ptr<Fr>(s.tmp), n_, ptr<Fr>(inj_tab_[j])));
        }
        HIPCHK(hipStreamSynchronize(st));
    }
    for (uint32_t k = 0; k < nb_commit_; k++) {
        CHK(qcp_c_[k].alloc(fn)); CHK(eqcp_[k].alloc(f4));
        HIPCHK(hipMemcpyAsync(s.wl.p, d->qcp[k], fn, hipMemcpyHostToDevice, st));
        CHK(inv_ntt_n(st, ptr<Fr>(s.wl), ptr<Fr>(qcp_c_[k])));
        CHK(coset_ntt_4n(st, ptr<Fr>(qcp_c_[k]), n_, ptr<Fr>(eqcp_[k])));
        scale_kernel<FRP><<<cdiv(n4_, POLY_THREADS), POLY_THREADS, 0, st>>>(ptr<Fr>(eqcp_[k]), fr_u64(1u << 5), n4_); KCHK();
        HIPCHK(hipStreamSynchronize(st));
    }
    {
        std::vector<Fr> wpow(n_);
        {
// ... 101 lines not shown

template <class FRP, class FPP, int CURVE_ID>
int CurveBackend<FRP, FPP, CURVE_ID>::wire_route(ProofRun& run) {
    Slot& s = run.s;
    hipStream_t st = run.st;
    const uint32_t n = n_;
    constexpr uint32_t DENSITY_UNKNOWN = 0xffffffffu;
    run.use_lag = run.measuring = false;
    if (!lagrange_possible() || hook_ || wires_lag_mode_ == 0) return APK_OK;
    const uint32_t seq = proof_seq_.fetch_add(1, std::memory_order_relaxed);
    uint32_t pm = wire_density_pm_.load(std::memory_order_relaxed);
    if (wires_lag_mode_ == 1) run.use_lag = true;
    else {
        run.measuring = pm == DENSITY_UNKNOWN || (seq & 15u) == 0;
        if (run.measuring) {
            uint32_t* d_cnt = ptr<uint32_t>(s.tail_flag) + 2;
            HIPCHK(hipMemsetAsync(d_cnt, 0, 4, st));
            MsmBatchArgs da{};
            da.batch = 3;
            const Fr* wires[3] = {run.dL, run.dR, run.dO};
            for (int j = 0; j < 3; j++) { da.scalars[j] = wires[j]; da.len[j] = n; }
            msm_density_kernel<FRP><<<dim3(cdiv(n, 256) < 512 ? cdiv(n, 256) : 512, 3), 256, 0, st>>>(da, msm_ctx_.win, d_cnt); KCHK();
            HIPCHK(hipMemcpyAsync(pin_host<uint32_t>(s.h_pinned, PIN_DENSITY), d_cnt, 4, hipMemcpyDeviceToHost, st));
        }
        if (pm == DENSITY_UNKNOWN) {
            HIPCHK(hipStreamSynchronize(st));
            pm = wire_route_finish(run);
        }
        run.use_lag = pm < 900u;
    }
    if (run.use_lag && !lagrange_ready()) run.use_lag = ensure_lagrange_table(st);
    return APK_OK;
}
template <class FRP, class FPP, int CURVE_ID>
uint32_t CurveBackend<FRP, FPP, CURVE_ID>::wire_route_finish(ProofRun& run) {
    const uint32_t count = *pin_host<const volatile uint32_t>(run.s.h_pinned, PIN_DENSITY);
    const uint32_t pm = (uint32_t)((uint64_t)count * 1000u / ((uint64_t)3 * n_ * msm_ctx_.W));
    wire_density_pm_.store(pm, std::memory_order_relaxed);
    run.measuring = false;
    return pm;
}

template <class FRP, class FPP, int CURVE_ID>
int CurveBackend<FRP, FPP, CURVE_ID>::round1_wires(ProofRun& run) {
    Slot& s = run.s;
    hipStream_t st = run.st;
    const uint32_t n = n_;
    const size_t fn = (size_t)n_ * sizeof(Fr);
    const Aff* hp = pin_host<Aff>(s.h_pinned, PIN_AFF);
    for (uint32_t k = 0; k < nb_commit_; k++) {
        const Fr* col = run.pi2[k];
        MsmBatchArgs a{};
        a.batch = 1; a.scalars[0] = col; a.len[0] = n; a.offset[0] = 0;
        CHK(commit(s, tab_lag_, 1, a));
        CHK(inv_ntt_n(st, col, ptr<Fr>(s.pi2_can[k])));
        {
            const Fr* cin = ptr<Fr>(s.pi2_can[k]); Fr* eout = ptr<Fr>(s.epi2[k]);
            CHK(coset_eval(st, 1, &cin, &n, &eout));
        }
        CHK(sync_results(s));
        run.bsb[k] = hp[0];
        run.cval[k] = Proto::hash_fr(run.bsb[k]);
        store_pt(run.out->bsb22[k], run.bsb[k]);
    }
    Fr* canon[3] = {ptr<Fr>(s.cl), ptr<Fr>(s.cr), ptr<Fr>(s.co)};
    const Fr* wires[3] = {run.dL, run.dR, run.dO};
    CHK(wire_route(run));
    const bool use_lag = run.use_lag;
    Fr* lagv[3] = {ptr<Fr>(s.wl), ptr<Fr>(s.wr), ptr<Fr>(s.wo)};
    if (use_lag)
        for (int j = 0; j < 3; j++) HIPCHK(hipMemcpyAsync(lagv[j], wires[j], fn, hipMemcpyDeviceToDevice, st));
    {
        const uint32_t lens[3] = {n, n, n};
        CHK(run_ntt_batch(st, 0, true, 3, wires, canon, lens, n, nullptr, nullptr, ptr<Fr>(scales_)));
    }
    {
        Blind3<FRP> b3{};
        for (int j = 0; j < 3; j++) {
            b3.p[j] = canon[j]; b3.b[j].v[0] = run.bl[2 * j]; b3.b[j].v[1] = run.bl[2 * j + 1];
            b3.lag[j] = use_lag ? lagv[j] : nullptr;
        }
        CHK((klaunch<Blind3K<FRP>, 256>(st, 3, 64, 0, b3, n, 2)));
    }
    const int fill = run.fill = tail_fill(s);
    if (fill) path(P_TAIL_FILL);
    {
        MsmBatchArgs a{};
        a.batch = 3;
        for (int j = 0; j < 3; j++) { a.scalars[j] = use_lag ? lagv[j] : canon[j]; a.len[j] = n + 2; a.offset[j] = 0; }
        a.plain = use_lag ? 1u : 0u;
        if (use_lag) path(P_LAGRANGE_WIRES);
        s.mark_acc = fill;
        const int rc = use_lag ? commit(s, tab_lag_, 1, a) : commit(s, tab_can_, 0, a);
        s.mark_acc = 0;
        CHK(rc);
    }
    if (!qk_direct_) {
        HIPCHK(hipMemcpyAsync(s.qk_lag.p, qk_lag_trace_.p, fn, hipMemcpyDeviceToDevice, st));
        if (nb_public_) HIPCHK(hipMemcpyAsync(s.qk_lag.p, run.pubv, (size_t)nb_public_ * sizeof(Fr), hipMemcpyHostToDevice, st));
        for (uint32_t k = 0; k < nb_commit_; k++)
            HIPCHK(hipMemcpyAsync(ptr<Fr>(s.qk_lag) + nb_public_ + cci_[k], &run.cval[k], sizeof(Fr), hipMemcpyHostToDevice, st));
        CHK(inv_ntt_n(st, ptr<Fr>(s.qk_lag), ptr<Fr>(s.qk_can)));
        CHK(coset_ntt_4n(st, ptr<Fr>(s.qk_can), n, ptr<Fr>(s.eqk)));
    }
    {
        Fr* ev[3] = {ptr<Fr>(s.el), ptr<Fr>(s.er), ptr<Fr>(s.eo)};
        const uint32_t lens[3] = {n + 2, n + 2, n + 2};
        if (wire_hook_ && !sc_.on()) {
            HIPCHK(hipStreamSynchronize(st));
            const void* cin[3] = {canon[0], canon[1], canon[2]};
            void* eout[3] = {ev[0], ev[1], ev[2]};
            hook_slot() = &s;
            const int rc = wire_hook_(wire_hook_user_, 3, cin, lens, eout);
            hook_slot() = nullptr;
            if (rc != APK_OK) { set_error("wire hook failed with %d", rc); return rc == APK_ERR_ARG ? APK_ERR_ARG : APK_ERR_STATE; }
        } else if (fill) {
            CHK(side_begin(s));
            CHK(run_ntt_batch(s.side, 1, false, 3, canon, ev, lens, n4_, ptr<Fr>(coset_pre_), nullptr, nullptr, 0, true));
            CHK(side_end(s));
        } else {
            CHK(coset_eval(st, 3, canon, lens, ev));
        }
    }
    CHK(sync_results(s));
    if (run.measuring) wire_route_finish(run);
    for (int j = 0; j < 3; j++) { run.lro[j] = hp[j]; store_pt(run.out->lro[j], run.lro[j]); }
    return APK_OK;
}

template <class FRP, class FPP, int CURVE_ID>
int CurveBackend<FRP, FPP, CURVE_ID>::round2_grand_product(ProofRun& run) {
    Slot& s = run.s;
    hipStream_t st = run.st;
    const uint32_t n = n_;
    const int fill = run.fill;
    {
        Fr* hfr = pin_host<Fr>(s.h_pinned, PIN_FR);
        const GpScan<FRP> g = poly_gp_scan<FRP>(ptr<Fr>(s.ratio), ptr<Fr>(s.tmp), ptr<Fr>(s.scan_tot), n);
        CHK(poly_gp_terms<FRP>(kl(), st, run.dL, run.dR, run.dO, (const Fr*)ptr<Fr>(s_lag_[0]), (const Fr*)ptr<Fr>(s_lag_[1]), (const Fr*)ptr<Fr>(s_lag_[2]),
                               (const Fr*)ptr<Fr>(tw_n_), n, run.beta * fr_u64(32), run.gamma, run.beta_u * fr_u64(32), run.beta_u2 * fr_u64(32), g));
        Fr* const tot_pin = pin_dev<Fr>(s.d_pinned, PIN_FR);
        Fr* const tot_out = tot_pin ? tot_pin : poly_gp_total_slot<FRP>(g, n);
        CHK(poly_gp_scans<FRP>(kl(), st, g, n, tot_out));
        if (!tot_pin) HIPCHK(hipMemcpyAsync(hfr, tot_out, sizeof(Fr), hipMemcpyDeviceToHost, st));
        CHK(sync_results(s));
        CHK(poly_gp_finish<FRP>(kl(), st, g, n, hfr[0], ptr<Fr>(s.zlag)));
    }
    CHK(inv_ntt_n(st, ptr<Fr>(s.zlag), ptr<Fr>(s.cz)));
    {
        Fr4<FRP> b{};
        b.v[0] = run.bl[6]; b.v[1] = run.bl[7]; b.v[2] = run.bl[8];
        CHK((klaunch<BlindK<FRP>, 256>(st, 1, 64, 0, ptr<Fr>(s.cz), n, b, 3)));
        MsmBatchArgs a{};
        a.batch = 1; a.scalars[0] = s.cz.p; a.len[0] = n + 3; a.offset[0] = 0;
        s.mark_acc = fill;
        const int rc = commit(s, tab_can_, 0, a);
        s.mark_acc = 0;
        CHK(rc);
    }
    if (fill) {
        CHK(side_begin(s));
        CHK(coset_ntt_4n(s.side, ptr<Fr>(s.cz), n + 3, ptr<Fr>(s.ez), true));
        CHK(side_end(s));
    } else {
        const Fr* cin = ptr<Fr>(s.cz); Fr* eout = ptr<Fr>(s.ez);
        const uint32_t zl = n + 3;
        CHK(coset_eval(st, 1, &cin, &zl, &eout));
        if (sc_.on() && sc_.glog == 3) {
            Fr* e2 = ptr<Fr>(s.eqk);
            CHK(coset_eval(st, 1, &cin, &zl, &e2, 1));
        }
    }
    CHK(sync_results(s));
    run.zcom = pin_host<Aff>(s.h_pinned, PIN_AFF)[0];
    store_pt(run.out->z, run.zcom);
    return APK_OK;
}

template <class FRP, class FPP, int CURVE_ID>
QuotientArgs<FRP> CurveBackend<FRP, FPP, CURVE_ID>::quotient_args(const ProofRun& run) {
    Slot& s = run.s;
    QuotientArgs<FRP> q{};
    q.l = ptr<Fr>(s.el); q.r = ptr<Fr>(s.er); q.o = ptr<Fr>(s.eo); q.z = ptr<Fr>(s.ez); q.qk = ptr<Fr>(s.eqk);
    if (qk_direct_) {
        q.qk = ptr<Fr>(eqk_trace_);
        q.nb_inject = (int)inj_row_.size();
        for (size_t j = 0; j < inj_row_.size(); j++) {
            const Fr written = j < nb_public_ ? run.pubv[j] : run.cval[j - nb_public_];
            q.inj_delta[j] = written - inj_trace_val_[j];
            q.inj_tab[j] = inj_row_[j] == 0 ? ptr<Fr>(l0_4_) : ptr<Fr>(inj_tab_[j]);
        }
    }
    q.ql = ptr<Fr>(eql_); q.qr = ptr<Fr>(eqr_); q.qm = ptr<Fr>(eqm_); q.qo = ptr<Fr>(eqo_);
    q.s1 = ptr<Fr>(es_[0]); q.s2 = ptr<Fr>(es_[1]); q.s3 = ptr<Fr>(es_[2]);
    q.x = ptr<Fr>(x4_); q.l0 = ptr<Fr>(l0_4_);
    q.nb_commit = (int)nb_commit_;
    for (uint32_t k = 0; k < nb_commit_; k++) { q.qcp[k] = ptr<Fr>(eqcp_[k]); q.pi2[k] = ptr<Fr>(s.epi2[k]); }
    const Fr c5 = fr_u64(1u << 5), c10 = fr_u64(1u << 10), c20 = fr_u64(1u << 20);
    q.alpha = run.alpha * c20; q.beta = run.beta * c5; q.gamma = run.gamma; q.beta_u = run.beta_u * c5; q.beta_u2 = run.beta_u2 * c5;
    q.alpha2 = run.alpha * run.alpha * c10;
    for (int k = 0; k < 4; k++) q.zh_inv[k] = zh_inv_[k] * c5;
    for (int j = 0; j < q.nb_inject; j++) q.inj_delta[j] = q.inj_delta[j] * c5;
    q.n4 = n4_;
    return q;
}

template <class FRP, class FPP, int CURVE_ID>
int CurveBackend<FRP, FPP, CURVE_ID>::round3_quotient(ProofRun& run) {
    Slot& s = run.s;
    hipStream_t st = run.st;
    const uint32_t n = n_;
    {
        QuotientArgs<FRP> q = quotient_args(run);
        if (!sc_.on()) {
            CHK((klaunch<QuotientK<FRP>, POLY_THREADS>(st, cdiv(n4_, POLY_THREADS), POLY_THREADS, 0, q, ptr<Fr>(s.quot))));
            CHK(run_ntt(st, 1, true, ptr<Fr>(s.quot), ptr<Fr>(s.hcan), n4_, n4_, nullptr, ptr<Fr>(coset_post_inv_), nullptr));
        } else {
            const uint32_t m = n4_ >> sc_.glog;
            q.n4 = m; q.sub_k = (uint32_t)sc_.k; q.sub_glog = (uint32_t)sc_.glog; q.zs = ptr<Fr>(s.eqk);
            quotient_kernel<FRP><<<cdiv(m, POLY_THREADS), POLY_THREADS, 0, st>>>(q, ptr<Fr>(s.quot)); KCHK();
            Fr* mine = ptr<Fr>(s.sc_gather) + (size_t)sc_.k * m;
            CHK(run_ntt(st, 1, true, ptr<Fr>(s.quot), mine, m, m, nullptr, ptr<Fr>(sc_.post), nullptr, sc_.glog));
            HIPCHK(hipStreamSynchronize(st));
            hook_slot() = &s;
            const int grc = sc_.hook(sc_.user, s.sc_gather.p, (size_t)m * sizeof(Fr));
            hook_slot() = nullptr;
            if (grc != APK_OK) { set_error("sub-coset gather hook failed with %d", grc); return grc == APK_ERR_ARG ? APK_ERR_ARG : APK_ERR_STATE; }
            SubMergeArgs<FRP> ma{};
            for (int e = 0; e < 8; e++) ma.rho_inv[e] = sc_.rho_inv[e];
            ma.m = m; ma.glog = (uint32_t)sc_.glog;
            subcoset_merge_kernel<FRP><<<cdiv(m, POLY_THREADS), POLY_THREADS, 0, st>>>(ma, ptr<Fr>(s.sc_gather), ptr<Fr>(coset_post_inv_), ptr<Fr>(s.hcan)); KCHK();
        }
        MsmBatchArgs a{};
        a.batch = 3;
        for (int j = 0; j < 3; j++) { a.scalars[j] = ptr<Fr>(s.hcan) + (size_t)j * (n + 2); a.len[j] = n + 2; a.offset[j] = 0; }
        CHK(commit(s, tab_can_, 0, a));
        s.epoch++;
        const uint32_t tail4 = (n4_ - 3 * (n + 2)) * (uint32_t)(sizeof(Fr) / 16);
        uint32_t* const flag_pin = pin_dev<uint32_t>(s.d_pinned, PIN_TAIL);
        CHK(poly_tail_nonzero(kl(), st, reinterpret_cast<const uint4*>(ptr<Fr>(s.hcan) + 3 * (size_t)(n + 2)), tail4, s.epoch,
                              flag_pin ? flag_pin : ptr<uint32_t>(s.tail_flag)));
        if (!flag_pin) HIPCHK(hipMemcpyAsync(pin_host<uint32_t>(s.h_pinned, PIN_TAIL), s.tail_flag.p, 4, hipMemcpyDeviceToHost, st));
    }
    CHK(sync_results(s));
    if (*pin_host<const volatile uint32_t>(s.h_pinned, PIN_TAIL) == s.epoch) {
        set_error("quotient is not a polynomial: the witness does not satisfy the circuit");
// ... 157 lines not shown
```

### algoplonk_amd/csrc/ffu.h

```cpp
#pragma once
#include "ff.h"
#include "ffu_asm.h"

template <class P>
struct FeU {
    static constexpr int L = P::UL;
    static constexpr int B = P::UB;
    static constexpr uint32_t MASK = (1u << B) - 1u;
    static constexpr int N = P::N;
    uint32_t l[L];

    APK_HD static FeU zero() {
        FeU r;
#pragma unroll
        for (int i = 0; i < L; i++) r.l[i] = 0;
        return r;
    }
    APK_HD static FeU one() {
        FeU r;
#pragma unroll
        for (int i = 0; i < L; i++) r.l[i] = P::uone(i);
        return r;
    }
    APK_HD bool is_zero() const {
// ... 229 lines not shown
    template <uint32_t K, uint32_t FB>
    APK_HD static constexpr uint32_t kp_s(int i) {
        uint32_t v = kp<K>(i);
        if (i < L - 1) v += FB << B;
        if (i > 0) v -= FB;
        return v;
    }
    template <uint32_t K, uint32_t FB>
    APK_HD static constexpr bool kp_s_valid() {
        for (int i = 1; i < L - 1; i++)
            if (kp<K>(i) + 1u < FB) return false;
        return kp<K>(L - 1) >= FB && ((uint64_t)(FB + 1) << B) <= (1ull << 32);
    }

    APK_HD static FeU add_s(const FeU& a, const FeU& b) {
        FeU r;
#pragma unroll
        for (int i = 0; i < L; i++) r.l[i] = a.l[i] + b.l[i];
        return r;
    }
    template <uint32_t K, uint32_t FB = 1>
    APK_HD static FeU sub_s(const FeU& a, const FeU& b) {
        static_assert(kp_s_valid<K, FB>(), "K*p has a limb too small to lend FB units");
        FeU r;
#pragma unroll
        for (int i = 0; i < L; i++) r.l[i] = a.l[i] - b.l[i] + kp_s<K, FB>(i);
        return r;
    }
    template <uint32_t K, uint32_t FB = 1>
    APK_HD static FeU neg_s(const FeU& a) {
        static_assert(kp_s_valid<K, FB>(), "K*p has a limb too small to lend FB units");
        FeU r;
#pragma unroll
        for (int i = 0; i < L; i++) r.l[i] = kp_s<K, FB>(i) - a.l[i];
        return r;
    }
    template <uint32_t K>
    APK_HD static FeU sub_n(const FeU& a, const FeU& b) {
        static_assert(kp_s_valid<K, 1>(), "K*p has a limb too small to lend one unit");
        FeU r;
        uint32_t carry = 0;
#pragma unroll
        for (int i = 0; i < L; i++) {
            uint32_t t = a.l[i] - b.l[i] + kp_s<K, 1>(i) + carry;
            carry = t >> B;
            r.l[i] = i == L - 1 ? t : (t & MASK);
        }
        return r;
    }

    APK_HD static FeU mul2_nr(const FeU& a, const FeU& b, const FeU& c, const FeU& d) {
        uint32_t m[L];
        FeU r;
        uint64_t acc = 0;
#pragma unroll
        for (int k = 0; k < L; k++) {
#pragma unroll
            for (int i = 0; i <= k; i++) {
                acc += (uint64_t)a.l[i] * b.l[k - i];
                acc += (uint64_t)c.l[i] * d.l[k - i];
            }
#pragma unroll
            for (int i = 0; i < k; i++) acc += (uint64_t)m[i] * P::umod(k - i);
            m[k] = ((uint32_t)acc * P::UINV) & MASK;
            acc += (uint64_t)m[k] * P::umod(0);
            acc >>= B;
        }
#pragma unroll
        for (int k = L; k < 2 * L - 1; k++) {
#pragma unroll
            for (int i = k - L + 1; i < L; i++) {
                acc += (uint64_t)a.l[i] * b.l[k - i];
                acc += (uint64_t)c.l[i] * d.l[k - i];
            }
#pragma unroll
            for (int i = k - L + 1; i < L; i++) acc += (uint64_t)m[i] * P::umod(k - i);
            r.l[k - L] = (uint32_t)acc & MASK;
            acc >>= B;
        }
        r.l[L - 1] = (uint32_t)acc;
        return r;
    }

    template <uint32_t K>
    APK_HD static FeU canon(const FeU& a) {
        FeU d;
        uint32_t borrow = 0;
#pragma unroll
        for (int i = 0; i < L; i++) {
            uint32_t t = a.l[i] - kp<K>(i) - borrow;
            borrow = t >> 31;
            d.l[i] = i == L - 1 ? t : (t & MASK);
        }
        FeU r;
#pragma unroll
        for (int i = 0; i < L; i++) r.l[i] = borrow ? a.l[i] : d.l[i];
        if constexpr (K > 1) return canon<K / 2>(r);
        else return r;
    }
    APK_HD static constexpr uint32_t cmod(int i) {
        uint32_t carry = 1, limb = 0;
        for (int j = 0; j <= i; j++) {
            const uint32_t t = (MASK - P::umod(j)) + carry;
            limb = t & MASK;
            carry = t >> B;
        }
        return limb;
    }
    template <uint32_t K>
    APK_HD static FeU reduce_2p(const FeU& a) {
        constexpr uint32_t T = P::umod(L - 1) + 1;
        constexpr int S = 62 - __builtin_clz(T);
        constexpr uint32_t C = (uint32_t)((1ull << S) / T);
        static_assert(4ull * (2 * K + 1) <= T - 1 && (uint64_t)2 * K * T <= (1ull << (S - 2)), "the estimate must stay within one of the quotient");
        static_assert((uint64_t)2 * K * T <= (1ull << 32), "the top limb of the input must fit its word");
        const uint32_t q = (uint32_t)(((uint64_t)a.l[L - 1] * C) >> S);
        FeU r;
        uint64_t acc = 0;
#pragma unroll
        for (int i = 0; i < L; i++) {
            acc += (uint64_t)q * cmod(i) + a.l[i];
            r.l[i] = (uint32_t)acc & MASK;
            acc >>= B;
        }
        return r;
    }
    APK_HD bool is_zero_mod_p() const {
        uint32_t z = 0, e = 0;
#pragma unroll
        for (int i = 0; i < L; i++) { z |= l[i]; e |= l[i] ^ P::umod(i); }
        return z == 0 || e == 0;
    }

    APK_HD static FeU unpack(const uint32_t* w) {
        FeU r;
#pragma unroll
        for (int i = 0; i < L; i++) {
            const int bit = i * B, j = bit >> 5, s = bit & 31;
            uint32_t v = j < N ? (w[j] >> s) : 0u;
            if (s + B > 32 && j + 1 < N) v |= w[j + 1] << (32 - s);
            r.l[i] = v & MASK;
        }
        return r;
    }
    APK_HD void pack(uint32_t* w) const {
#pragma unroll
        for (int j = 0; j < N; j++) {
            uint32_t v = 0;
#pragma unroll
            for (int i = 0; i < L; i++) {
                const int lo = i * B - j * 32;
                if (lo > -B && lo < 32) v |= lo >= 0 ? (l[i] << lo) : (l[i] >> (-lo));
            }
            w[j] = v;
        }
    }

    APK_HD static FeU from_fe(const Fe<P>& x) {
        FeU c;
#pragma unroll
        for (int i = 0; i < L; i++) c.l[i] = P::uconv_in(i);
        return mul(unpack(x.l), c);
    }
    APK_HD Fe<P> to_fe() const {
        FeU c;
#pragma unroll
// ... 12 lines not shown
```

### algoplonk_amd/csrc/kernels_poly.h

```cpp
#pragma once
#include "ff.h"
#include "ffu.h"

namespace apk {

constexpr int POLY_THREADS = 256;
constexpr int SCAN_PER_THREAD = 8;
constexpr int SCAN_BLOCK = POLY_THREADS * SCAN_PER_THREAD;

template <class FR>
struct Fr4 { Fe<FR> v[4]; };

template <class FR>
__global__ void fill_zero_kernel(Fe<FR>* p, uint32_t count) {
    uint32_t i = blockIdx.x * blockDim.x + threadIdx.x;
    if (i < count) p[i] = Fe<FR>::zero();
}

template <class FR>
struct BlindK {
    static __device__ __forceinline__ void run(Fe<FR>* p, uint32_t n, Fr4<FR> b, int d) {
        int i = threadIdx.x;
        if (i < d) {
            p[i] = p[i] - b.v[i];
            p[n + i] = b.v[i];
        }
    }
};
template <class FR>
__global__ void blind_kernel(Fe<FR>* p, uint32_t n, Fr4<FR> b, int d) { BlindK<FR>::run(p, n, b, d); }
template <class FR>
struct Blind3 {
    Fe<FR>* p[3];
    Fr4<FR> b[3];
    Fe<FR>* lag[3];
};
template <class FR>
struct Blind3K {
    static __device__ __forceinline__ void run(Blind3<FR> a, uint32_t n, int d) {
        int i = threadIdx.x;
        Fe<FR>* p = a.p[blockIdx.x];
        if (i < d) {
            const Fe<FR> v = a.b[blockIdx.x].v[i];
            if (p) {
                p[i] = p[i] - v;
                p[n + i] = v;
            }
            if (a.lag[blockIdx.x]) a.lag[blockIdx.x][n + i] = v;
        }
    }
};
template <class FR>
__global__ void blind3_kernel(Blind3<FR> a, uint32_t n, int d) { Blind3K<FR>::run(a, n, d); }

template <class FR>
struct MulK {
    static __device__ __forceinline__ void run(Fe<FR>* out, const Fe<FR>* a, const Fe<FR>* b, uint32_t count) {
        wave_priority<APK_PRIO_FR>();
        uint32_t i = blockIdx.x * blockDim.x + threadIdx.x;
        if (i < count) out[i] = a[i] * b[i];
    }
};
template <class FR>
__global__ void mul_kernel(Fe<FR>* out, const Fe<FR>* a, const Fe<FR>* b, uint32_t count) { MulK<FR>::run(out, a, b, count); }

template <class FR>
struct GpTermsK {
    static __device__ __forceinline__ void run(const Fe<FR>* __restrict__ L, const Fe<FR>* __restrict__ R,
                                                                const Fe<FR>* __restrict__ O, const Fe<FR>* __restrict__ S1,
                                                                const Fe<FR>* __restrict__ S2, const Fe<FR>* __restrict__ S3,
                                                                const Fe<FR>* __restrict__ tw, uint32_t n, Fe<FR> beta,
                                                                Fe<FR> gamma, Fe<FR> beta_u, Fe<FR> beta_u2,
                                                                Fe<FR>* __restrict__ num, Fe<FR>* __restrict__ den) {
        wave_priority<APK_PRIO_FR>();
        using Fr = Fe<FR>;
        uint32_t i = blockIdx.x * blockDim.x + threadIdx.x;
        if (i >= n) return;
        using U = FeU<FR>;
        static_assert(U::HEADROOM >= 64, "factors below 4 r");
        auto ld = [](const Fr* p, uint32_t k) { Fr v = p[k]; return U::unpack(v.l); };
        Fr wf = i < n / 2 ? tw[i] : Fr::neg(tw[i - n / 2]);
        const U w = U::unpack(wf.l), gm = U::unpack(gamma.l), b = U::unpack(beta.l), bu = U::unpack(beta_u.l), bu2 = U::unpack(beta_u2.l);
        const U l = U::add_n(ld(L, i), gm), r = U::add_n(ld(R, i), gm), o = U::add_n(ld(O, i), gm);
        U nu = U::mul_nr(U::add_n(l, U::mul_nr(b, w)), U::add_n(r, U::mul_nr(bu, w)));
        nu = U::mul_nr(nu, U::add_n(o, U::mul_nr(bu2, w)));
        U de = U::mul_nr(U::add_n(l, U::mul_nr(b, ld(S1, i))), U::add_n(r, U::mul_nr(b, ld(S2, i))));
        de = U::mul_nr(de, U::add_n(o, U::mul_nr(b, ld(S3, i))));
        Fr on, od;
        U::template canon<1>(nu).pack(on.l);
        U::template canon<1>(de).pack(od.l);
        num[i] = on;
        den[i] = od;
    }
};
// ... 113 lines not shown
    }
};
template <class FR>
__global__ void __launch_bounds__(POLY_THREADS) gp_scan_block_kernel(GpScan<FR> g, uint32_t count) { GpScanBlockK<FR>::run(g, count); }
template <class FR>
struct GpScanTotalsK {
    static __device__ __forceinline__ void run(GpScan<FR> g, uint32_t nblocks, Fe<FR>* __restrict__ total_out) {
        wave_priority<APK_PRIO_FR>();
        Fe<FR> total = scan_totals_body<FR, OpMul>(g.tot[blockIdx.x], nblocks);
        if (blockIdx.x == 1 && threadIdx.x == POLY_THREADS - 1) *total_out = total;
    }
};
template <class FR>
__global__ void __launch_bounds__(POLY_THREADS) gp_scan_totals_kernel(GpScan<FR> g, uint32_t nblocks, Fe<FR>* __restrict__ total_out) { GpScanTotalsK<FR>::run(g, nblocks, total_out); }
template <class FR>
struct GpFinishK {
    static __device__ __forceinline__ void run(GpScan<FR> g, uint32_t n, Fe<FR> den_total_inv, Fe<FR>* __restrict__ z) {
        wave_priority<APK_PRIO_FR>();
        using Fr = Fe<FR>;
        uint32_t k = blockIdx.x * blockDim.x + threadIdx.x;
        if (k >= n) return;
        if (k == 0) { z[0] = Fr::one(); return; }
        Fr np = g.tot[0][(k - 1) / SCAN_BLOCK] * g.data[0][k - 1];
        Fr ds = g.tot[1][(n - 1 - k) / SCAN_BLOCK] * g.data[1][k];
        z[k] = np * (ds * den_total_inv);
    }
};
template <class FR>
__global__ void __launch_bounds__(POLY_THREADS) gp_finish_kernel(GpScan<FR> g, uint32_t n, Fe<FR> den_total_inv, Fe<FR>* __restrict__ z) { GpFinishK<FR>::run(g, n, den_total_inv, z); }

template <class FR, class OP>
struct ScanApplyK {
    static __device__ __forceinline__ void run(const Fe<FR>* __restrict__ data, uint32_t count, bool rev,
                                                                  const Fe<FR>* __restrict__ block_excl,
                                                                  Fe<FR>* __restrict__ out, int shift) {
        wave_priority<APK_PRIO_FR>();
        using Fr = Fe<FR>;
        uint32_t i = blockIdx.x * blockDim.x + threadIdx.x;
        if (i >= count) return;
        Fr v = OP::apply(block_excl[i / SCAN_BLOCK], data[scan_idx(i, count, rev)]);
        if (shift) {
            if (i + 1 < count) out[i + 1] = v;
            if (i == 0) out[0] = OP::template identity<Fr>();
        } else {
            out[scan_idx(i, count, rev)] = v;
        }
    }
};
template <class FR, class OP>
__global__ void __launch_bounds__(POLY_THREADS) scan_apply_kernel(const Fe<FR>* __restrict__ data, uint32_t count, bool rev,
                                                                  const Fe<FR>* __restrict__ block_excl,
                                                                  Fe<FR>* __restrict__ out, int shift) { ScanApplyK<FR, OP>::run(data, count, rev, block_excl, out, shift); }

constexpr int QK_INJECT_MAX = 6;
template <class FR>
struct QuotientArgs {
    const Fe<FR>*l, *r, *o, *z, *qk;
    const Fe<FR>*ql, *qr, *qm, *qo, *s1, *s2, *s3;
    const Fe<FR>*x, *l0;
    const Fe<FR>* qcp[2];
    const Fe<FR>* pi2[2];
    int nb_commit;
    int nb_inject;
    const Fe<FR>* inj_tab[QK_INJECT_MAX];
    Fe<FR> inj_delta[QK_INJECT_MAX];
    Fe<FR> alpha, beta, gamma, beta_u, beta_u2, alpha2;
    Fe<FR> zh_inv[4];
    uint32_t n4;
    const Fe<FR>* zs;
    uint32_t sub_k, sub_glog;
};

template <class FR>
struct QuotientK {
    static __device__ __forceinline__ void run(QuotientArgs<FR> a, Fe<FR>* __restrict__ out) {
        wave_priority<APK_PRIO_FR>();
        using Fr = Fe<FR>;
        using U = FeU<FR>;
        static_assert(U::HEADROOM >= 64, "a lazy sum below 17 r times a canonical factor must stay below 2 r");
        const uint32_t jj = blockIdx.x * blockDim.x + threadIdx.x;
        if (jj >= a.n4) return;
        const uint32_t i = (jj << a.sub_glog) + a.sub_k;
        auto ld = [](const Fr* p, uint32_t k) { Fr v = p[k]; return U::unpack(v.l); };
        auto cst = [](const Fr& v) { return U::unpack(v.l); };
        const U l = ld(a.l, jj), r = ld(a.r, jj), o = ld(a.o, jj), z = ld(a.z, jj);
        uint32_t is;
        const Fr* zsp = a.z;
        if (a.sub_glog <= 2) is = jj + (4u >> a.sub_glog);
        else { is = jj + (a.sub_k + 4u >= 8u ? 1u : 0u); zsp = a.zs; }
        if (is >= a.n4) is -= a.n4;
        const U zs = ld(zsp, is);
        U gate = U::add_n(U::mul_nr(ld(a.ql, i), l), U::mul_nr(ld(a.qr, i), r));
        gate = U::add_n(gate, U::mul_nr(ld(a.qm, i), U::mul_nr(l, r)));
        gate = U::add_n(gate, U::mul_nr(ld(a.qo, i), o));
        gate = U::add_n(gate, ld(a.qk, i));
        for (int k = 0; k < a.nb_commit; k++) gate = U::add_n(gate, U::mul_nr(ld(a.qcp[k], i), ld(a.pi2[k], jj)));
        for (int j = 0; j < a.nb_inject; j++) gate = U::add_n(gate, U::mul_nr(cst(a.inj_delta[j]), ld(a.inj_tab[j], i)));
        const U gm = cst(a.gamma), beta = cst(a.beta);
        const U lg = U::add_n(l, gm), rg = U::add_n(r, gm), og = U::add_n(o, gm);
        const U x = ld(a.x, i);
        U pa = U::mul_nr(zs, U::add_n(lg, U::mul_nr(beta, ld(a.s1, i))));
        pa = U::mul_nr(pa, U::add_n(rg, U::mul_nr(beta, ld(a.s2, i))));
        pa = U::mul_nr(pa, U::add_n(og, U::mul_nr(beta, ld(a.s3, i))));
        U pb = U::mul_nr(z, U::add_n(lg, U::mul_nr(beta, x)));
        pb = U::mul_nr(pb, U::add_n(rg, U::mul_nr(cst(a.beta_u), x)));
        pb = U::mul_nr(pb, U::add_n(og, U::mul_nr(cst(a.beta_u2), x)));
        const U perm = U::mul_nr(cst(a.alpha), U::template sub_k<2>(pa, pb));
        const Fr one_r = Fr::one();
        const U one = U::unpack(one_r.l);
        const U loc = U::mul_nr(cst(a.alpha2), U::mul_nr(ld(a.l0, i), U::template sub_k<1>(z, one)));
        const U num = U::add_n(U::add_n(gate, perm), loc);
        const U res = U::template canon<1>(U::mul_nr(cst(a.zh_inv[i & 3]), num));
        Fr w;
        res.pack(w.l);
        out[jj] = w;
    }
};
template <class FR>
__global__ void __launch_bounds__(POLY_THREADS) quotient_kernel(QuotientArgs<FR> a, Fe<FR>* __restrict__ out) { QuotientK<FR>::run(a, out); }

template <class FR>
struct SubMergeArgs { Fe<FR> rho_inv[8]; uint32_t m, glog; };
template <class FR>
__global__ void __launch_bounds__(POLY_THREADS) subcoset_merge_kernel(SubMergeArgs<FR> a, const Fe<FR>* __restrict__ part, const Fe<FR>* __restrict__ post,
                                                                      Fe<FR>* __restrict__ out) {
    wave_priority<APK_PRIO_FR>();
    using Fr = Fe<FR>;
    using U = FeU<FR>;
    static_assert(U::HEADROOM >= 64, "sums of 8 products below 2 r each");
    const uint32_t cp = blockIdx.x * blockDim.x + threadIdx.x;
    if (cp >= a.m) return;
    const uint32_t G = 1u << a.glog;
    U v[8];
    for (uint32_t k = 0; k < G; k++) { Fr x = part[(size_t)k * a.m + cp]; v[k] = U::unpack(x.l); }
    for (uint32_t t = 0; t < G; t++) {
        U acc = v[0];
        for (uint32_t k = 1; k < G; k++) {
            const uint32_t e = (k * t) & (G - 1u);
            acc = U::add_n(acc, e ? U::mul_nr(U::unpack(a.rho_inv[e].l), v[k]) : v[k]);
        }
        const size_t c = (size_t)t * a.m + cp;
        Fr pw = post[c];
        const U res = U::template canon<1>(U::mul_nr(U::unpack(pw.l), acc));
        Fr w;
        res.pack(w.l);
        out[c] = w;
    }
}

template <class FR>
__global__ void __launch_bounds__(POLY_THREADS) scale_kernel(Fe<FR>* __restrict__ p, Fe<FR> c, uint32_t count) {
    uint32_t i = blockIdx.x * blockDim.x + threadIdx.x;
    if (i < count) p[i] = p[i] * c;
}

constexpr int EVAL_MAX = 12;
template <class FR>
struct EvalArgs {
    const Fe<FR>* f[EVAL_MAX];
    const Fe<FR>* pw[EVAL_MAX];
    uint32_t len[EVAL_MAX];
    int count;
};
constexpr int EVAL_PER_THREAD = 8;
constexpr int EVAL_BLOCK = POLY_THREADS * EVAL_PER_THREAD;

template <class FR>
struct EvalPartialK {
    static __device__ __forceinline__ void run(EvalArgs<FR> a, const Fe<FR>* __restrict__ pw,
                                                                    uint32_t nblocks, Fe<FR>* __restrict__ partial) {
        wave_priority<APK_PRIO_FR>();
        using Fr = Fe<FR>;
        __shared__ Fr sm[POLY_THREADS];
        const int p = blockIdx.y;
        const uint32_t t = threadIdx.x;
        const Fr* f = a.f[p];
        const Fr* __restrict__ pwp = a.pw[p] ? a.pw[p] : pw;
        const uint32_t len = a.len[p];
        using U = FeU<FR>;
        static_assert(U::HEADROOM >= 64 && EVAL_PER_THREAD * 2 <= 16, "8 products below 2 r each");
        U accu = U::zero();
        for (int k = 0; k < EVAL_PER_THREAD; k++) {
            uint32_t i = blockIdx.x * EVAL_BLOCK + k * POLY_THREADS + t;
            if (i < len) { Fr a0 = f[i], b0 = pwp[i]; accu = U::add_n(accu, U::mul_nr(U::unpack(a0.l), U::unpack(b0.l))); }
        }
        Fr acc;
        U::template canon<1>(U::template reduce_2p<8>(accu)).pack(acc.l);
        sm[t] = acc;
        __syncthreads();
        for (uint32_t d = POLY_THREADS / 2; d >= 1; d >>= 1) {
            if (t < d) { acc = acc + sm[t + d]; sm[t] = acc; }
            __syncthreads();
        }
        if (t == 0) partial[p * nblocks + blockIdx.x] = acc;
    }
};
template <class FR>
__global__ void __launch_bounds__(POLY_THREADS) eval_partial_kernel(EvalArgs<FR> a, const Fe<FR>* __restrict__ pw,
                                                                    uint32_t nblocks, Fe<FR>* __restrict__ partial) { EvalPartialK<FR>::run(a, pw, nblocks, partial); }

template <class FR>
struct EvalFinalK {
    static __device__ __forceinline__ void run(const Fe<FR>* __restrict__ partial, uint32_t nblocks,
                                                                  Fe<FR>* __restrict__ result) {
        wave_priority<APK_PRIO_FR>();
        using Fr = Fe<FR>;
        __shared__ Fr sm[POLY_THREADS];
        const int p = blockIdx.x;
        const uint32_t t = threadIdx.x;
        Fr acc = Fr::zero();
        for (uint32_t i = t; i < nblocks; i += POLY_THREADS) acc = acc + partial[p * nblocks + i];
        sm[t] = acc;
        __syncthreads();
        for (uint32_t d = POLY_THREADS / 2; d >= 1; d >>= 1) {
            if (t < d) { acc = acc + sm[t + d]; sm[t] = acc; }
            __syncthreads();
        }
        if (t == 0) result[p] = acc;
    }
};
template <class FR>
__global__ void __launch_bounds__(POLY_THREADS) eval_final_kernel(const Fe<FR>* __restrict__ partial, uint32_t nblocks,
                                                                  Fe<FR>* __restrict__ result) { EvalFinalK<FR>::run(partial, nblocks, result); }

template <class FR>
struct DerivePowers { const Fe<FR>* in[2]; Fe<FR>* out[2]; int inverse[2]; };
template <class FR>
struct DerivePowersK {
    static __device__ __forceinline__ void run(DerivePowers<FR> a, const Fe<FR>* __restrict__ twu, uint32_t n, uint32_t count) {
        wave_priority<APK_PRIO_FR>();
        using Fr = Fe<FR>;
        using U = FeU<FR>;
        const uint32_t i = blockIdx.x * blockDim.x + threadIdx.x;
        if (i >= count) return;
        const int p = blockIdx.y;
        uint32_t e = i & (n - 1u);
        if (a.inverse[p]) e = (n - e) & (n - 1u);
        const bool neg = e >= n / 2;
        Fr w = twu[e & (n / 2 - 1u)], v = a.in[p][i];
        U r = U::template canon<1>(U::mul_nr(U::unpack(w.l), U::unpack(v.l)));
        Fr o;
        r.pack(o.l);
        if (neg) o = Fr::neg(o);
        a.out[p][i] = o;
    }
};
template <class FR>
__global__ void __launch_bounds__(POLY_THREADS) derive_powers_kernel(DerivePowers<FR> a, const Fe<FR>* __restrict__ twu, uint32_t n, uint32_t count) { DerivePowersK<FR>::run(a, twu, n, count); }

constexpr int LC_MAX = 20;
template <class FR>
struct LinCombArgs {
    const Fe<FR>* f[LC_MAX];
    uint32_t len[LC_MAX];
    Fe<FR> coef[LC_MAX];
    int count;
    uint32_t out_len;
};

template <class FR>
struct LincombK {
    static __device__ __forceinline__ void run(LinCombArgs<FR> a, Fe<FR>* __restrict__ out) {
        wave_priority<APK_PRIO_FR>();
        using Fr = Fe<FR>;
        using U = FeU<FR>;
        static_assert(U::HEADROOM >= 64 && LC_MAX * 2 <= 64, "the sum of LC_MAX products below 2 r each must stay below 64 r");
        uint32_t i = blockIdx.x * blockDim.x + threadIdx.x;
        if (i >= a.out_len) return;
        U acc = U::zero();
        for (int k = 0; k < a.count; k++)
            if (i < a.len[k]) { Fr v = a.f[k][i]; acc = U::add_n(acc, U::mul_nr(U::unpack(a.coef[k].l), U::unpack(v.l))); }
        const U res = U::template canon<1>(U::template reduce_2p<32>(acc));
        Fr w;
        res.pack(w.l);
        out[i] = w;
    }
};
template <class FR>
__global__ void __launch_bounds__(POLY_THREADS) lincomb_kernel(LinCombArgs<FR> a, Fe<FR>* __restrict__ out) { LincombK<FR>::run(a, out); }

template <class FR>
struct DivFinishK {
    static __device__ __forceinline__ void run(const Fe<FR>* __restrict__ suffix,
                                                                  const Fe<FR>* __restrict__ zinv_pw, uint32_t len,
                                                                  Fe<FR>* __restrict__ q) {
        wave_priority<APK_PRIO_FR>();
        uint32_t j = blockIdx.x * blockDim.x + threadIdx.x;
        if (j + 1 >= len) return;
        q[j] = suffix[j + 1] * zinv_pw[j + 1];
    }
};
template <class FR>
__global__ void __launch_bounds__(POLY_THREADS) div_finish_kernel(const Fe<FR>* __restrict__ suffix,
                                                                  const Fe<FR>* __restrict__ zinv_pw, uint32_t len,
                                                                  Fe<FR>* __restrict__ q) { DivFinishK<FR>::run(suffix, zinv_pw, len, q); }

constexpr int KZG_QUOT_MAX = 2;
template <class FR>
struct KzgQuotBatch {
    const Fe<FR>* f[KZG_QUOT_MAX];
    const Fe<FR>* pw[KZG_QUOT_MAX];
    const Fe<FR>* pwi[KZG_QUOT_MAX];
    Fe<FR>* tmp[KZG_QUOT_MAX];
    Fe<FR>* tot[KZG_QUOT_MAX];
    Fe<FR>* q[KZG_QUOT_MAX];
    uint32_t len[KZG_QUOT_MAX];
};
template <class FR>
struct KzgScanBlockBatchK {
    static __device__ __forceinline__ void run(KzgQuotBatch<FR> b) {
        const uint32_t p = blockIdx.y;
        if (blockIdx.x * (uint32_t)SCAN_BLOCK >= b.len[p]) return;
        wave_priority<APK_PRIO_FR>();
        const Fe<FR>* __restrict__ f = b.f[p];
        const Fe<FR>* __restrict__ pw = b.pw[p];
        scan_block_body_ld<FR, OpAdd>([f, pw](uint32_t m) { return f[m] * pw[m]; }, b.tmp[p], b.len[p], true, b.tot[p]);
    }
};
template <class FR>
struct KzgScanTotalsBatchK {
    static __device__ __forceinline__ void run(KzgQuotBatch<FR> b) {
        const uint32_t p = blockIdx.x;
        ScanTotalsK<FR, OpAdd>::run(b.tot[p], (b.len[p] + SCAN_BLOCK - 1) / SCAN_BLOCK);
    }
};
template <class FR>
struct KzgDivFinishBatchK {
    static __device__ __forceinline__ void run(KzgQuotBatch<FR> b) {
        wave_priority<APK_PRIO_FR>();
        const uint32_t p = blockIdx.y, len = b.len[p];
        const uint32_t j = blockIdx.x * blockDim.x + threadIdx.x;
        if (j + 1 >= len) return;
        const Fe<FR> suffix = OpAdd::apply(b.tot[p][(len - 2 - j) / SCAN_BLOCK], b.tmp[p][j + 1]);
        b.q[p][j] = suffix * b.pwi[p][j + 1];
    }
};

template <int DUMMY>
struct TailNonzeroK {
    static __device__ __forceinline__ void run(const uint4* __restrict__ words, uint32_t count4, uint32_t epoch, uint32_t* __restrict__ flag) {
        uint32_t acc = 0;
        for (uint32_t i = blockIdx.x * blockDim.x + threadIdx.x; i < count4; i += gridDim.x * blockDim.x) {
            const uint4 v = words[i];
            acc |= v.x | v.y | v.z | v.w;
        }
        if (__ballot(acc != 0) != 0 && (threadIdx.x & 63) == 0) *reinterpret_cast<volatile uint32_t*>(flag) = epoch;
    }
};
template <int DUMMY>
__global__ void __launch_bounds__(256) tail_nonzero_kernel(const uint4* __restrict__ words, uint32_t count4, uint32_t epoch, uint32_t* __restrict__ flag) { TailNonzeroK<DUMMY>::run(words, count4, epoch, flag); }

template <class FR>
struct ShiftDownK {
    static __device__ __forceinline__ void run(const Fe<FR>* __restrict__ f, uint32_t len, Fe<FR>* __restrict__ q) {
// ... 9 lines not shown
```

### algoplonk_amd/csrc/selftest_ops.h

```cpp
#pragma once
#include <string.h>
#include <type_traits>

#include "ec.h"

namespace apk {

enum { SELFTEST_OK = 0, SELFTEST_UNKNOWN_OP = 1, SELFTEST_NO_UNSAT = 2 };

template <class P, class = void> struct HasUnsat : std::false_type {};
template <class P> struct HasUnsat<P, std::void_t<decltype(P::UL)>> : std::true_type {};

template <class P>
APK_HD int fe_op_t(int op, const void* a, const void* b, void* out) {
    using F = Fe<P>;
    F x, y, r;
    memcpy(&x, a, sizeof x);
    if (b) memcpy(&y, b, sizeof y); else y = F::zero();
    switch (op) {
        case 0: r = F::add(x, y); break;
        case 1: r = F::sub(x, y); break;
        case 2: r = F::mul(x, y); break;
        case 3: r = F::inv(x); break;
        case 4: r = F::neg(x); break;
// ... 2 lines not shown
                using U = FeU<P>;
                U ux = U::from_fe(x), uy = U::from_fe(y);
                r = (op == 10 ? U::mul(ux, uy) : op == 11 ? U::add(ux, uy) : op == 12 ? U::sub(ux, uy) : U::neg(ux)).to_fe();
                break;
            } else {
                return SELFTEST_NO_UNSAT;
            }
        case 14:
            if constexpr (HasUnsat<P>::value) {
                using U = FeU<P>;
                F ratio = F::zero();
                ratio.l[0] = 1u << (U::B * U::L - 32 * F::N);
                const U w = U::unpack(F::mul(y, F::to_mont(ratio)).l);
                U u = U::unpack(x.l), v = U::unpack(y.l);
                for (int i = 0; i < 10; i++) {
                    const U t = U::mul_nr(w, v);
                    const U nu = U::add_n(u, t);
                    v = U::template sub_k<2>(u, t);
                    u = nu;
                }
                U::template canon<16>(u).pack(r.l);
                break;
            } else {
                return SELFTEST_NO_UNSAT;
            }
        default: return SELFTEST_UNKNOWN_OP;
    }
    memcpy(out, &r, sizeof r);
    return SELFTEST_OK;
}

template <class P>
APK_HD int feu_op_t(int op, const uint32_t* in, uint32_t* out) {
    if constexpr (HasUnsat<P>::value) {
        using U = FeU<P>;
        constexpr int L = U::L;
        U a, b, c, d, r = U::zero();
        for (int i = 0; i < L; i++) { a.l[i] = in[i]; b.l[i] = in[L + i]; c.l[i] = in[2 * L + i]; d.l[i] = in[3 * L + i]; }
        switch (op) {
            case 0: r = U::reduce_once(a); break;
            case 1: r = U::add(a, b); break;
            case 2: r = U::sub(a, b); break;
            case 3: r = U::neg(a); break;
            case 4: r = U::mul_nr(a, b); break;
            case 5: r = U::mul(a, b); break;
            case 6: r = U::sqr_nr(a); break;
            case 7: r = U::sqr(a); break;
            case 8: r = U::mul2_nr(a, b, c, d); break;
            case 9: r = U::add_n(a, b); break;
            case 10: r = U::triple_n(a); break;
            case 11: r = U::template sub2_k<4>(a, b, c); break;
            case 12: r = U::template sub_k<1>(a, b); break;
            case 13: r = U::template sub_k<2>(a, b); break;
            case 14: r = U::template sub_k<4>(a, b); break;
            case 15: r = U::template sub_k<6>(a, b); break;
            case 16: r = U::template neg_k<1>(a); break;
            case 17: r = U::template neg_k<2>(a); break;
            case 18: r = U::template neg_k<4>(a); break;
            case 19: r = U::template canon<1>(a); break;
            case 20: r = U::template canon<2>(a); break;
            case 21: r = U::template canon<4>(a); break;
            case 22: r = U::template canon<8>(a); break;
            case 23: r = U::template canon<16>(a); break;
            case 24: r = U::template canon<32>(a); break;
            case 25: r.l[0] = a.is_zero_mod_p() ? 1u : 0u; break;
            case 26: r = U::unpack(in); break;
            case 27: a.pack(r.l); break;
            case 28: { Fe<P> x; memcpy(&x, in, sizeof x); r = U::from_fe(x); break; }
            case 29: { const Fe<P> x = a.to_fe(); memcpy(r.l, &x, sizeof x); break; }
            case 40: r = U::add_s(a, b); break;
            case 41: r = U::template sub_s<2>(a, b); break;
            case 42: r = U::template neg_s<2>(a); break;
            case 43: r = U::template sub_n<2>(a, b); break;
            case 44: r = U::template reduce_2p<4>(a); break;
            case 45: r = U::template reduce_2p<8>(a); break;
            case 46: r = U::template reduce_2p<32>(a); break;
            case 47: r = U::template canon<1>(U::template reduce_2p<32>(a)); break;
            case 48:
                r.l[0] = U::mul_takes(a.l[0], a.l[1]) ? 1u : 0u;
                r.l[1] = U::mul2_takes(a.l[0], a.l[1], a.l[2], a.l[3]) ? 1u : 0u;
                r.l[2] = U::sqr_takes(a.l[0]) ? 1u : 0u;
                r.l[3] = (uint32_t)U::COLUMN_ROOM;
                break;
            default: return SELFTEST_UNKNOWN_OP;
        }
        for (int i = 0; i < L; i++) out[i] = r.l[i];
        return SELFTEST_OK;
    } else {
        return SELFTEST_NO_UNSAT;
    }
}

template <class U>
APK_HD bool feu_scaled_le(const U& v, uint32_t sv, uint32_t k) {
    constexpr int L = U::L;
    uint64_t x[U::L], y[U::L], cx = 0, cy = 0;
    for (int i = 0; i < L; i++) {
        const uint64_t tx = (uint64_t)sv * v.l[i] + cx, ty = (uint64_t)k * U::template kp<1>(i) + cy;
        x[i] = i == L - 1 ? tx : (tx & U::MASK); cx = tx >> U::B;
        y[i] = i == L - 1 ? ty : (ty & U::MASK); cy = ty >> U::B;
    }
    for (int i = L - 1; i >= 0; i--)
        if (x[i] != y[i]) return x[i] < y[i];
    return true;
}
template <class XU>
APK_HD bool in_lazy_class(const XU& pt) {
    using U = decltype(pt.X);
    for (int i = 0; i < U::L - 1; i++)
        if ((pt.X.l[i] | pt.Y.l[i] | pt.ZZ.l[i] | pt.ZZZ.l[i]) > U::MASK) return false;
    return feu_scaled_le(pt.X, 10, 51) && feu_scaled_le(pt.Y, 1, 4) && feu_scaled_le(pt.ZZ, 10, 14) && feu_scaled_le(pt.ZZZ, 10, 14);
}

constexpr int LAZY_CHAIN_STEPS = 320;

template <class FRP, class FPP>
APK_HD int g1_op_t(int op, const void* p, const void* q, void* out) {
    using A = Affine<FPP>;
    using X = XYZZ<FPP>;
    A a, b, r;
    memcpy(&a, p, sizeof a);
    switch (op) {
        case 0: {
            memcpy(&b, q, sizeof b);
            X acc = X::from_affine(a);
            acc.madd(b);
            r = acc.to_affine();
            break;
        }
        case 1: {
            memcpy(&b, q, sizeof b);
            X acc = X::dbl_affine(a);
            acc.madd(a, true);
            X other = X::dbl_affine(b);
            other.madd(b, true);
            acc.add(other);
            r = acc.to_affine();
            break;
        }
        case 2: r = X::dbl(X::from_affine(a)).to_affine(); break;
        case 3: {
            Fe<FRP> s;
            memcpy(&s, q, sizeof s);
            s = Fe<FRP>::from_mont(s);
            X acc = X::inf();
            for (int w = Fe<FRP>::N - 1; w >= 0; w--)
                for (int bit = 31; bit >= 0; bit--) {
                    acc = X::dbl(acc);
                    if ((s.l[w] >> bit) & 1u) acc.madd(a);
                }
            r = acc.to_affine();
            break;
        }
        case 12: case 13: {
            using XU = XYZZ<FPP, FeU<FPP>>;
            memcpy(&b, q, sizeof b);
            const Affine<FPP, FeU<FPP>> pa = unpack_affine<FPP>(to_table_record<FPP>(a)), pb = unpack_affine<FPP>(to_table_record<FPP>(b)),
                                        pinf = Affine<FPP, FeU<FPP>>::inf();
            constexpr int script[17][2] = {{0, 0}, {0, 0}, {0, 1}, {0, 1}, {1, 0}, {1, 0}, {0, 0}, {1, 0}, {0, 1}, {1, 1}, {1, 1},
                                           {2, 0}, {0, 0}, {1, 0}, {1, 0}, {0, 1}, {0, 0}};
            XU acc = XU::inf();
            bool flipped = false, unit_z = false;
            for (const auto& st : script) {
                const auto& pt = st[0] == 0 ? pa : st[0] == 1 ? pb : pinf;
                if (op == 12) acc.madd_lazy(pt, st[1] != 0, flipped, unit_z); else acc.madd(pt, st[1] != 0);
            }
// ... 107 lines not shown
```

### algoplonk_amd/plonk.py

```python
from __future__ import annotations

import ctypes as C
import os
from dataclasses import dataclass, field
from typing import List, Optional, Sequence

from . import ecc, frontend
from . import _lib
from ._lib import lib, check
from .setup import SRS


@dataclass
class VerifyingKey:
    curve: ecc.ID
    Size: int
    SizeInv: int
    Generator: int
    CosetShift: int
    NbPublicVariables: int
    Ql: ecc.Point
    Qr: ecc.Point
    Qm: ecc.Point
    Qo: ecc.Point
# ... 2 lines not shown
    Qcp: List[ecc.Point]
    CommitmentConstraintIndexes: List[int]
    KzgG1: ecc.Point
    tau: Optional[int] = None
    KzgG2: Optional[bytes] = None

    def raw(self) -> "_lib.VerifyingKey":
        cv = self.curve
        if not self.KzgG2:
            raise ValueError("verifying key carries no G2 points")
        v = _lib.VerifyingKey()
        v.curve, v.n, v.nb_public, v.nb_commitments = cv.abi, self.Size, self.NbPublicVariables, len(self.Qcp)

        def put(slot, P):
            b = cv.g1_to_bytes(P)
            C.memmove(slot, b, len(b))

        for name, P in (("ql", self.Ql), ("qr", self.Qr), ("qm", self.Qm), ("qo", self.Qo), ("qk", self.Qk), ("g1", self.KzgG1)):
            put(getattr(v, name), P)
        for j in range(3):
            put(v.s[j], self.S[j])
        for k, P in enumerate(self.Qcp):
            put(v.qcp[k], P)
            v.commitment_constraint_index[k] = self.CommitmentConstraintIndexes[k]
        w = 4 * cv.fp_bytes
        for j in range(2):
            C.memmove(v.g2[j], self.KzgG2[j * w: (j + 1) * w], w)
        return v


class ProvingKey:

    def __init__(self, curve: ecc.ID, ctx: int, n: int, nb_public: int):
        self.curve = curve
        self._ctx = C.c_void_p(ctx)
        self.n = n
        self.nb_public = nb_public

    @property
    def ctx(self) -> C.c_void_p:
        if not self._ctx:
            raise RuntimeError("proving key was closed")
        return self._ctx

    def close(self) -> None:
        if self._ctx:
            lib.apk_ctx_destroy(self._ctx)
            self._ctx = C.c_void_p(None)

    def __del__(self):
        try:
            self.close()
        except Exception:
            pass

    def msm(self, scalars: Sequence[int], basis: int = 0) -> ecc.Point:
        cv = self.curve
        buf = cv.fr_vector(scalars)
        out = C.create_string_buffer(2 * cv.fp_bytes)
        check(lib.apk_msm_g1(self.ctx, basis, buf, len(scalars), out))
        return cv.g1_from_bytes(out.raw)

    def ntt(self, values: Sequence[int], which: int = 0, inverse: bool = False, coset: bool = False) -> List[int]:
        cv = self.curve
        buf = C.create_string_buffer(cv.fr_vector(values), len(values) * 32)
        check(lib.apk_ntt(self.ctx, which, int(inverse), int(coset), buf))
        return cv.fr_vector_decode(buf.raw)

    def stats(self, reset: bool = False) -> "_lib.Stats":
        st = _lib.Stats()
        check(lib.apk_stats_read(self.ctx, C.byref(st), int(reset)))
        return st

    def enable_stats(self, on: bool = True) -> None:
        check(lib.apk_stats_enable(self.ctx, int(on)))

    @property
    def msm_window(self) -> int:
        return lib.apk_ctx_msm_window(self.ctx)

    def paths(self, reset: bool = False) -> dict:
        pc = _lib.PathCounts()
        check(lib.apk_paths_read(self.ctx, C.byref(pc), int(reset)))
        return pc.as_dict()


@dataclass
class Proof:
    curve: ecc.ID
    raw: "_lib.Proof"

    def _pt(self, slot) -> ecc.Point:
        return self.curve.g1_from_bytes(bytes(slot))

    def _fr(self, slot) -> int:
        return self.curve.fr_from_mont_bytes(bytes(slot))

    @property
    def LRO(self): return [self._pt(self.raw.lro[i]) for i in range(3)]
    @property
    def Z(self): return self._pt(self.raw.z)
    @property
    def H(self): return [self._pt(self.raw.h[i]) for i in range(3)]
    @property
    def Bsb22Commitments(self): return [self._pt(self.raw.bsb22[i]) for i in range(self.raw.nb_commitments)]
    @property
    def BatchedProofH(self): return self._pt(self.raw.batched_h)
    @property
    def ClaimedValues(self): return [self._fr(self.raw.claimed_values[i]) for i in range(6 + self.raw.nb_commitments)]
    @property
    def ZShiftedOpeningH(self): return self._pt(self.raw.zshift_h)
    @property
    def ZShiftedOpeningClaimedValue(self): return self._fr(self.raw.zshift_value)
    @property
    def challenges(self): return {k: self._fr(getattr(self.raw, k)) for k in ("gamma", "beta", "alpha", "zeta", "gamma_kzg")}


def Setup(ccs: frontend.ConstraintSystem, srs: SRS, device: int = 0, msm_window: int = 0, slots: int = 1):
    cv = srs.curve
    tr = frontend.build_trace(ccs)
    if tr.n != srs.n:
        raise ValueError("SRS sized for n=%d, circuit needs n=%d" % (srs.n, tr.n))
    cols = [cv.fr_vector(c) for c in (tr.ql, tr.qr, tr.qm, tr.qo, tr.qk)]
    perm = (C.c_int64 * len(tr.perm))(*tr.perm)
    d = _lib.CircuitDesc()
    d.curve, d.device, d.n = cv.abi, device, tr.n
    nbc = len(ccs.commitments)
    if nbc > _lib.MAX_COMMITMENTS:
        raise ValueError("at most %d BSB22 commitments" % _lib.MAX_COMMITMENTS)
    if nbc and not srs.g1_lagrange:
        raise ValueError("circuits with BSB22 commitments need the Lagrange SRS")
    d.nb_public, d.nb_commitments = ccs.GetNbPublicVariables(), nbc
    qcp_cols = [cv.fr_vector(c) for c in tr.qcp]
    for k in range(nbc):
        d.qcp[k] = C.cast(C.c_char_p(qcp_cols[k]), C.c_void_p)
        d.commitment_constraint_index[k] = ccs.commitments[k][1]
    keep = [srs.g1, srs.g1_lagrange] + cols + qcp_cols
    d.srs_g1 = C.cast(C.c_char_p(srs.g1), C.c_void_p)
    d.srs_g1_lagrange = C.cast(C.c_char_p(srs.g1_lagrange), C.c_void_p) if srs.g1_lagrange else None
    d.ql, d.qr, d.qm, d.qo, d.qk = (C.cast(C.c_char_p(c), C.c_void_p) for c in cols)
    d.perm = C.cast(perm, C.c_void_p)
    d.msm_window, d.slots = msm_window, slots
    ctx = C.c_void_p()
    check(lib.apk_ctx_create(C.byref(d), C.byref(ctx)))
    del keep
    pk = ProvingKey(cv, ctx.value, tr.n, ccs.GetNbPublicVariables())
    raw = _lib.Vk()
    check(lib.apk_ctx_get_vk(pk.ctx, C.byref(raw)))
    P = lambda slot: cv.g1_from_bytes(bytes(slot))
    F = lambda slot: cv.fr_from_mont_bytes(bytes(slot))
    vk = VerifyingKey(
        curve=cv, Size=tr.n, SizeInv=F(raw.size_inv), Generator=F(raw.generator), CosetShift=F(raw.coset_shift),
        NbPublicVariables=ccs.GetNbPublicVariables(), Ql=P(raw.ql), Qr=P(raw.qr), Qm=P(raw.qm), Qo=P(raw.qo), Qk=P(raw.qk),
        S=[P(raw.s[i]) for i in range(3)], Qcp=[P(raw.qcp[k]) for k in range(nbc)],
        CommitmentConstraintIndexes=[ccs.commitments[k][1] for k in range(nbc)],
        KzgG1=cv.g1_from_bytes(srs.g1[: 2 * cv.fp_bytes]), tau=srs.tau, KzgG2=srs.g2)
    return pk, vk


class VerificationError(RuntimeError):
    pass


def Verify(proof: "Proof", vk: VerifyingKey, public_witness: frontend.Witness) -> None:
    cv = vk.curve
    public = public_witness.Public().public
    if len(public) != vk.NbPublicVariables:
# ... 183 lines not shown
```

### include/apk.h

```cpp
#ifndef APK_H
#define APK_H

#include <stddef.h>
#include <stdint.h>

#ifdef __cplusplus
extern "C" {
#endif

#define APK_ABI_VERSION 5

#define APK_BN254 0
#define APK_BLS12_381 1

#define APK_OK 0
#define APK_ERR_ARG 1
#define APK_ERR_HIP 2
#define APK_ERR_STATE 3
#define APK_ERR_WITNESS 4
#define APK_ERR_VERIFY 5

#define APK_FR_BYTES 32
#define APK_G1_MAX_BYTES 96
#define APK_G2_MAX_BYTES 192
// ... 250 lines not shown
#define APK_POLY_GRAND_PRODUCT 0
#define APK_POLY_SCAN 1
#define APK_POLY_QUOTIENT 2
#define APK_POLY_MERGE 3
#define APK_POLY_EVAL 4
#define APK_POLY_LINCOMB 5
#define APK_POLY_DERIVE_POWERS 6
#define APK_POLY_KZG_QUOTIENT 7
#define APK_POLY_BLIND 8
#define APK_POLY_BLIND3 9
#define APK_POLY_TAIL 10
#define APK_POLY_KZG_QUOTIENT2 11
#define APK_POLY_VECS 32
#define APK_POLY_FRS 24
#define APK_POLY_INTS 8
#define APK_POLY_OUTS 6
typedef struct {
    const void* vec[APK_POLY_VECS];
    uint64_t len[APK_POLY_VECS];
    uint8_t fr[APK_POLY_FRS][32];
    int64_t iv[APK_POLY_INTS];
    void* out[APK_POLY_OUTS];
    uint64_t out_len[APK_POLY_OUTS];
} apk_poly_args;
int apk_device_poly_op(int curve, int op, int device, const apk_poly_args* args);
int apk_g1_sum(int curve, const void* points, uint64_t count, void* out);

int apk_host_alloc(int device, size_t bytes, void** ptr);
int apk_host_free(void* ptr);
int apk_host_register(void* ptr, size_t bytes);
int apk_host_unregister(void* ptr);

int apk_device_alloc(apk_ctx* ctx, size_t bytes, void** d_ptr);
int apk_device_free(apk_ctx* ctx, void* d_ptr);
int apk_device_upload(apk_ctx* ctx, void* d_dst, const void* src, size_t bytes);
int apk_device_download(apk_ctx* ctx, void* dst, const void* d_src, size_t bytes);
int apk_device_copy(apk_ctx* ctx, void* d_dst, const void* d_src, size_t bytes);

typedef struct {
    double msm_accumulate_ms;
    uint64_t msm_accumulate_launches;
    uint64_t msm_pairs;
    double msm_total_ms;
    uint64_t msm_batches;
    double ntt_ms;
    uint64_t ntt_elements;
    double prove_ms;
    uint64_t proofs;
    double round_ms[4];
    double host_lincomb_ms;
    double msm_sort_ms;
    double msm_tail_ms;
} apk_stats;
int apk_stats_enable(apk_ctx* ctx, int enable);
int apk_stats_read(apk_ctx* ctx, apk_stats* out, int reset);

typedef struct {
    uint64_t proofs;
    uint64_t msm_batches;
    uint64_t msm_sort_two_level;
    uint64_t msm_sort_two_level_by_load;
    uint64_t msm_sort_fused;
    uint64_t msm_lean_tail;
    uint64_t msm_rowcol_serial;
    uint64_t msm_combine_quad;
    uint64_t msm_small_units;
    uint64_t msm_one_launch;
    uint64_t msm_lagrange_wires;
    uint64_t ntt_sequences;
    uint64_t ntt_radix4;
    uint64_t ntt_radix4_by_load;
    uint64_t tail_fill_proofs;
    uint64_t host_lincomb_pooled;
    uint64_t msm_units_by_load;
    uint64_t host_inputs;
    uint64_t gang_proofs;
    uint64_t gang_msm_launches;
    uint64_t gang_ntt_launches;
    uint64_t gang_kernel_launches;
    uint64_t forms_by_device_load;
    uint64_t msm_inplace;
} apk_path_counts;
int apk_paths_read(apk_ctx* ctx, apk_path_counts* out, int reset);

typedef struct {
    uint32_t contexts;
    uint32_t max_streams;
    uint32_t streams_in_use, streams_peak;
    uint32_t proofs_in_flight, proofs_peak;
    uint32_t waiting;
    uint32_t device_wide;
} apk_device_sched;
int apk_device_sched_read(int device, apk_device_sched* out, int reset);

#define APK_HWQ_UNSET (-1)
#define APK_HWQ_UNREADABLE (-2)
typedef struct {
    int32_t hw_queues_found;
    int32_t hw_queues_left;
    int32_t hw_queues_need;
    int32_t hw_queues_written;
    int32_t hw_queues_now;
    int32_t first_hip_call;
    int32_t hw_queues_at_first_hip;
    int32_t reserved;
} apk_runtime;
int apk_runtime_read(apk_runtime* out);

#ifdef __cplusplus
}
#endif
#endif
```

Baseline: 555.9.

## Add lazy-reduction dot products to quotient, eval and lincomb kernels; optional coset deferral

Adds a Montgomery dot-product primitive that sums several limb products per column before a single reduction. The quotient numerator, polynomial evaluation and linear-combination kernels now use it in place of chained mul_nr and add_n calls. Uniform arguments are broadcast through readfirstlane so they can live in scalar registers. A new knob, off by default, lets the wire coset NTTs be deferred and batched with Z, and a new path counter API reports when that happens. The change trades fewer reductions for larger column accumulators, which may raise register pressure in these kernels.

Measured after the change: 563.4, median of 6. +1.4%, better.

```diff
diff --git a/algoplonk_amd/_lib.py b/algoplonk_amd/_lib.py
--- a/algoplonk_amd/_lib.py
+++ b/algoplonk_amd/_lib.py
@@ -24,7 +24,7 @@
     "apk_device_fe_op", "apk_device_g1_op", "apk_host_feu_op", "apk_device_feu_op", "apk_feu_shape", "apk_device_poly_op",
     "apk_device_alloc", "apk_device_free", "apk_device_upload", "apk_device_download",
     "apk_host_alloc", "apk_host_free", "apk_host_register", "apk_host_unregister",
-    "apk_stats_enable", "apk_stats_read", "apk_paths_read",
+    "apk_stats_enable", "apk_stats_read", "apk_paths_read", "apk_paths_read_more",
     "apk_ctx_set_wire_hook", "apk_coset_ntt_device",
     "apk_comm_create", "apk_comm_destroy", "apk_comm_rank", "apk_comm_world", "apk_comm_barrier", "apk_comm_max_f64", "apk_comm_bind",
     "apk_comm_transport", "apk_msm_g1_sharded", "apk_comm_split_begin", "apk_comm_split_end", "apk_comm_serve", "apk_comm_set_compute",
@@ -136,6 +136,14 @@
 
     def as_dict(self) -> dict:
         return {n: int(getattr(self, n)) for n in self._names + self._later}
+
+
+class PathCountsMore(C.Structure):
+    _names = ["coset_deferred"]
+    _fields_ = [(n, C.c_uint64) for n in _names] + [("reserved", C.c_uint64 * 7)]
+
+    def as_dict(self) -> dict:
+        return {n: int(getattr(self, n)) for n in self._names}
 
 
 class DeviceSched(C.Structure):
@@ -254,6 +262,8 @@
     lib.apk_stats_enable.argtypes = [vp, i32]
     lib.apk_stats_read.argtypes = [vp, C.POINTER(Stats), i32]
     lib.apk_paths_read.argtypes = [vp, C.POINTER(PathCounts), i32]
+    if hasattr(lib, "apk_paths_read_more"):
+        lib.apk_paths_read_more.argtypes = [vp, C.POINTER(PathCountsMore), i32]
     if hasattr(lib, "apk_device_sched_read"):
         lib.apk_device_sched_read.argtypes = [i32, C.POINTER(DeviceSched), i32]
     if hasattr(lib, "apk_runtime_read"):
diff --git a/algoplonk_amd/csrc/apk_api.cpp b/algoplonk_amd/csrc/apk_api.cpp
--- a/algoplonk_amd/csrc/apk_api.cpp
+++ b/algoplonk_amd/csrc/apk_api.cpp
@@ -548,6 +548,7 @@
     return APK_OK;
 }
 int apk_paths_read(apk_ctx* ctx, apk_path_counts* out, int reset) { NEED_CTX(); if (!out) { set_error("null out"); return APK_ERR_ARG; } return ctx->be->paths_read(out, reset); }
+int apk_paths_read_more(apk_ctx* ctx, apk_path_counts_more* out, int reset) { NEED_CTX(); if (!out) { set_error("null out"); return APK_ERR_ARG; } return ctx->be->paths_read_more(out, reset); }
 int apk_runtime_read(apk_runtime* out) {
     if (!out) { set_error("null out"); return APK_ERR_ARG; }
     memset(out, 0, sizeof *out);
@@ -634,7 +635,7 @@
 
 int apk_device_feu_op(int curve, int field, int op, int device, uint64_t count, const void* in, void* out) {
     if (count && (!in || !out)) { set_error("null argument"); return APK_ERR_ARG; }
-    if (!seam_args(curve, count, (op >= 0 && op <= 29) || (op >= 40 && op <= 48), op, "unsaturated")) return APK_ERR_ARG;
+    if (!seam_args(curve, count, (op >= 0 && op <= 29) || (op >= 40 && op <= 48) || (op >= 50 && op <= 62), op, "unsaturated")) return APK_ERR_ARG;
     if (count == 0) return APK_OK;
     runtime_checkpoint();
     return curve == APK_BN254 ? feu_op_device_bn254(device, field, op, count, in, out) : feu_op_device_bls12381(device, field, op, count, in, out);
diff --git a/algoplonk_amd/csrc/backend.h b/algoplonk_amd/csrc/backend.h
--- a/algoplonk_amd/csrc/backend.h
+++ b/algoplonk_amd/csrc/backend.h
@@ -56,6 +56,7 @@
     virtual int stats_enable(int enable) = 0;
     virtual int stats_read(apk_stats* out, int reset) = 0;
     virtual int paths_read(apk_path_counts* out, int reset) = 0;
+    virtual int paths_read_more(apk_path_counts_more* out, int reset) = 0;
 };
 
 int g1_mul_batch_bn254(int device, const void* base, const void* scalars, uint64_t count, void* out);
diff --git a/algoplonk_amd/csrc/backend_impl.h b/algoplonk_amd/csrc/backend_impl.h
--- a/algoplonk_amd/csrc/backend_impl.h
+++ b/algoplonk_amd/csrc/backend_impl.h
@@ -59,6 +59,7 @@
         int open_pair = env_int("APK_OPEN_PAIR", 1, 0, 1);
         int lin_early_h = env_int("APK_LIN_EARLY_H", 1, 0, 1);
         int tail_fill = env_int("APK_TAIL_FILL", 1, 0, 2);
+        int coset_defer = env_int("APK_COSET_DEFER", 0, -1, 1);
     };
     static const ProverKnobs& prover_knobs() { static const ProverKnobs k{}; return k; }
 
@@ -184,6 +185,15 @@
                    P_ONE_LAUNCH, P_LAGRANGE_WIRES, P_NTT_SEQ, P_NTT_R4, P_NTT_R4_LOAD, P_TAIL_FILL, P_LINCOMB_POOL, P_UNIT_LOADED, P_HOST_INPUTS, P_GANG_PROOFS, P_GANG_MSM, P_GANG_NTT, P_GANG_KERNELS, P_DEVICE_LOAD, P_MSM_INPLACE, P_COUNT };
     std::atomic<uint64_t> paths_[P_COUNT] = {};
     void path(PathIdx i) { paths_[i].fetch_add(1, std::memory_order_relaxed); }
+    enum PathMoreIdx { PM_COSET_DEFER, PM_COUNT };
+    std::atomic<uint64_t> paths_more_[PM_COUNT] = {};
+    int paths_read_more(apk_path_counts_more* out, int reset) override {
+        static_assert(sizeof(apk_path_counts_more) >= PM_COUNT * sizeof(uint64_t), "apk_path_counts_more holds every counter");
+        memset(out, 0, sizeof *out);
+        uint64_t* o = reinterpret_cast<uint64_t*>(out);
+        for (int i = 0; i < PM_COUNT; i++) o[i] = reset ? paths_more_[i].exchange(0, std::memory_order_relaxed) : paths_more_[i].load(std::memory_order_relaxed);
+        return APK_OK;
+    }
     bool device_load_over(int thr, bool* foreign = nullptr) {
         int own = 0;
         const int dev = gate_.load(&own);
@@ -435,6 +445,11 @@
                 hipEventCreateWithFlags(&s.ev_side, hipEventDisableTiming) != hipSuccess) return 0;
         }
         return s.ev_acc && s.ev_side ? on : 0;
+    }
+    bool coset_defer() {
+        if (hook_ || wire_hook_ || sc_.on()) return false;
+        const int k = prover_knobs().coset_defer;
+        return k >= 0 ? k != 0 : slots_.size() > 2 && device_load_over(1);
     }
     int side_begin(Slot& s) { HIPCHK(hipStreamWaitEvent(s.side, s.ev_acc, 0)); return APK_OK; }
     int side_end(Slot& s) { HIPCHK(hipEventRecord(s.ev_side, s.side)); s.side_pending = true; return APK_OK; }
@@ -1482,6 +1497,7 @@
         uint8_t gamma_raw[32], beta_raw[32], alpha_raw[32], zeta_raw[32], gk_raw[32];
         typename Proto::KeyPoints key;
         int fill = 0;
+        bool defer = false;
         bool use_lag = false, measuring = false;
         std::chrono::steady_clock::time_point t_start, t_phase;
         double phase_ms[4] = {0, 0, 0, 0}, lincomb_ms = 0;
@@ -1749,8 +1765,9 @@
         }
         CHK((klaunch<Blind3K<FRP>, 256>(st, 3, 64, 0, b3, n, 2)));
     }
-    const int fill = run.fill = tail_fill(s);
+    const int fill = run.fill = prover_knobs().coset_defer == 1 ? 0 : tail_fill(s);
     if (fill) path(P_TAIL_FILL);
+    run.defer = !fill && coset_defer();
     {
         MsmBatchArgs a{};
         a.batch = 3;
@@ -1785,7 +1802,7 @@
             CHK(side_begin(s));
             CHK(run_ntt_batch(s.side, 1, false, 3, canon, ev, lens, n4_, ptr<Fr>(coset_pre_), nullptr, nullptr, 0, true));
             CHK(side_end(s));
-        } else {
+        } else if (!run.defer) {
             CHK(coset_eval(st, 3, canon, lens, ev));
         }
     }
@@ -1829,6 +1846,13 @@
         CHK(side_begin(s));
         CHK(coset_ntt_4n(s.side, ptr<Fr>(s.cz), n + 3, ptr<Fr>(s.ez), true));
         CHK(side_end(s));
+    } else if (run.defer) {
+        const Fr* cin[4] = {ptr<Fr>(s.cl), ptr<Fr>(s.cr), ptr<Fr>(s.co), ptr<Fr>(s.cz)};
+        Fr* eout[4] = {ptr<Fr>(s.el), ptr<Fr>(s.er), ptr<Fr>(s.eo), ptr<Fr>(s.ez)};
+        const uint32_t lens[4] = {n + 2, n + 2, n + 2, n + 3};
+        static_assert(NTT_MAX_BATCH >= 4, "the three wires and Z share one launch sequence");
+        CHK(coset_eval(st, 4, cin, lens, eout));
+        paths_more_[PM_COSET_DEFER].fetch_add(1, std::memory_order_relaxed);
     } else {
         const Fr* cin = ptr<Fr>(s.cz); Fr* eout = ptr<Fr>(s.ez);
         const uint32_t zl = n + 3;
diff --git a/algoplonk_amd/csrc/ffu.h b/algoplonk_amd/csrc/ffu.h
--- a/algoplonk_amd/csrc/ffu.h
+++ b/algoplonk_amd/csrc/ffu.h
@@ -335,6 +335,99 @@
         return r;
     }
 
+    APK_HD static constexpr bool dot_takes(uint64_t K, uint64_t fa, uint64_t fb) {
+        return K >= 1 && K * L * fa * fb < COLUMN_ROOM && (fa << B) <= (1ull << 32) && (fb << B) <= (1ull << 32);
+    }
+    APK_HD static constexpr bool dot_fuses(uint64_t K, uint64_t fa, uint64_t fb) {
+        return dot_takes(K, fa, fb) && K * L * fa * fb + L + 1 <= COLUMN_ROOM;
+    }
+    APK_HD static constexpr uint32_t dot_max_factor(uint64_t K) {
+        uint32_t f = 1;
+        while (dot_takes(K, f + 1, 1)) f++;
+        return f;
+    }
+    static_assert(dot_fuses(1, 1, 1) == mul_takes(1, 1) && dot_fuses(2, 1, 1) == mul2_takes(1, 1, 1, 1), "one budget for all products");
+
+    struct Cols { uint64_t c[2 * L - 1]; };
+    APK_HD static Cols cols_zero() {
+        Cols s;
+#pragma unroll
+        for (int k = 0; k < 2 * L - 1; k++) s.c[k] = 0;
+        return s;
+    }
+    APK_HD static void cols_mac(Cols& s, const FeU& a, const FeU& b) {
+#pragma unroll
+        for (int i = 0; i < L; i++) {
+#pragma unroll
+            for (int j = 0; j < L; j++) s.c[i + j] += (uint64_t)a.l[i] * b.l[j];
+        }
+    }
+    template <int K, uint32_t FA = 1, uint32_t FB = 1>
+    APK_HD static FeU cols_reduce(const Cols& s) {
+        static_assert(dot_takes(K, FA, FB), "the K products of a column must fit 64 bits");
+        constexpr bool FUSED = dot_fuses(K, FA, FB);
+        uint32_t m[L];
+        FeU r;
+        uint64_t acc = 0;
+#pragma unroll
+        for (int k = 0; k < 2 * L - 1; k++) {
+            const uint64_t prod = s.c[k];
+            if constexpr (FUSED) acc += prod;
+#pragma unroll
+            for (int i = k < L ? 0 : k - L + 1; i < L && i < k; i++) acc += (uint64_t)m[i] * P::umod(k - i);
+            const uint32_t low32 = FUSED ? (uint32_t)acc : (uint32_t)acc + (uint32_t)prod;
+            if (k < L) {
+                m[k] = (low32 * P::UINV) & MASK;
+                acc += (uint64_t)m[k] * P::umod(0);
+            } else {
+                r.l[k - L] = low32 & MASK;
+            }
+            if constexpr (FUSED) {
+                acc >>= B;
+            } else {
+                const uint32_t low = ((uint32_t)acc & MASK) + ((uint32_t)prod & MASK);
+                acc = (acc >> B) + (prod >> B) + (low >> B);
+            }
+        }
+        r.l[L - 1] = (uint32_t)acc;
+        return r;
+    }
+
+    template <int K, uint32_t FA = 1, uint32_t FB = 1>
+    APK_HD static FeU dot_nr(const FeU* a, const FeU* b) {
+        static_assert(dot_takes(K, FA, FB), "the K products of a column must fit 64 bits");
+        if constexpr (!dot_fuses(K, FA, FB)) {
+            Cols s = cols_zero();
+#pragma unroll
+            for (int t = 0; t < K; t++) cols_mac(s, a[t], b[t]);
+            return cols_reduce<K, FA, FB>(s);
+        } else {
+            uint32_t m[L];
+            FeU r;
+            uint64_t acc = 0;
+#pragma unroll
+            for (int k = 0; k < 2 * L - 1; k++) {
+                const int lo = k < L ? 0 : k - L + 1, hi = k < L ? k : L - 1;
+#pragma unroll
+                for (int i = lo; i <= hi; i++) {
+#pragma unroll
+                    for (int t = 0; t < K; t++) acc += (uint64_t)a[t].l[i] * b[t].l[k - i];
+                }
+#pragma unroll
+                for (int i = lo; i <= hi && i < k; i++) acc += (uint64_t)m[i] * P::umod(k - i);
+                if (k < L) {
+                    m[k] = ((uint32_t)acc * P::UINV) & MASK;
+                    acc += (uint64_t)m[k] * P::umod(0);
+                } else {
+                    r.l[k - L] = (uint32_t)acc & MASK;
+                }
+                acc >>= B;
+            }
+            r.l[L - 1] = (uint32_t)acc;
+            return r;
+        }
+    }
+
     template <uint32_t K>
     APK_HD static FeU canon(const FeU& a) {
         FeU d;
diff --git a/algoplonk_amd/csrc/kernels_poly.h b/algoplonk_amd/csrc/kernels_poly.h
--- a/algoplonk_amd/csrc/kernels_poly.h
+++ b/algoplonk_amd/csrc/kernels_poly.h
@@ -10,6 +10,21 @@
 
 template <class FR>
 struct Fr4 { Fe<FR> v[4]; };
+
+template <class FR>
+__device__ __forceinline__ Fe<FR> wave_uniform(const Fe<FR>& v) {
+    Fe<FR> r;
+#pragma unroll
+    for (int i = 0; i < Fe<FR>::N; i++) r.l[i] = __builtin_amdgcn_readfirstlane(v.l[i]);
+    return r;
+}
+__device__ __forceinline__ uint32_t wave_uniform(uint32_t v) { return __builtin_amdgcn_readfirstlane(v); }
+template <class T>
+__device__ __forceinline__ T* wave_uniform(T* p) {
+    const uint64_t v = reinterpret_cast<uint64_t>(p);
+    const uint32_t lo = wave_uniform((uint32_t)v), hi = wave_uniform((uint32_t)(v >> 32));
+    return reinterpret_cast<T*>((uint64_t)lo | ((uint64_t)hi << 32));
+}
 
 template <class FR>
 __global__ void fill_zero_kernel(Fe<FR>* p, uint32_t count) {
@@ -289,7 +304,7 @@
         if (jj >= a.n4) return;
         const uint32_t i = (jj << a.sub_glog) + a.sub_k;
         auto ld = [](const Fr* p, uint32_t k) { Fr v = p[k]; return U::unpack(v.l); };
-        auto cst = [](const Fr& v) { return U::unpack(v.l); };
+        auto cst = [](const Fr& v) { return U::unpack(wave_uniform(v).l); };
         const U l = ld(a.l, jj), r = ld(a.r, jj), o = ld(a.o, jj), z = ld(a.z, jj);
         uint32_t is;
         const Fr* zsp = a.z;
@@ -297,12 +312,32 @@
         else { is = jj + (a.sub_k + 4u >= 8u ? 1u : 0u); zsp = a.zs; }
         if (is >= a.n4) is -= a.n4;
         const U zs = ld(zsp, is);
-        U gate = U::add_n(U::mul_nr(ld(a.ql, i), l), U::mul_nr(ld(a.qr, i), r));
-        gate = U::add_n(gate, U::mul_nr(ld(a.qm, i), U::mul_nr(l, r)));
-        gate = U::add_n(gate, U::mul_nr(ld(a.qo, i), o));
-        gate = U::add_n(gate, ld(a.qk, i));
-        for (int k = 0; k < a.nb_commit; k++) gate = U::add_n(gate, U::mul_nr(ld(a.qcp[k], i), ld(a.pi2[k], jj)));
-        for (int j = 0; j < a.nb_inject; j++) gate = U::add_n(gate, U::mul_nr(cst(a.inj_delta[j]), ld(a.inj_tab[j], i)));
+        U extra = ld(a.qk, i);
+        if (a.nb_commit == 2) {
+            const U qc[2] = {ld(a.qcp[0], i), ld(a.qcp[1], i)}, pv[2] = {ld(a.pi2[0], jj), ld(a.pi2[1], jj)};
+            static_assert(U::dot_fuses(2, 1, 1), "qcp and pi2 normalised");
+            extra = U::add_n(extra, U::template dot_nr<2>(qc, pv));
+        } else if (a.nb_commit == 1) {
+            extra = U::add_n(extra, U::mul_nr(ld(a.qcp[0], i), ld(a.pi2[0], jj)));
+        }
+        for (int j = 0; j < a.nb_inject; j += 3) {
+            const int left = a.nb_inject - j;
+            if (left >= 3) {
+                const U dl[3] = {cst(a.inj_delta[j]), cst(a.inj_delta[j + 1]), cst(a.inj_delta[j + 2])};
+                const U tb[3] = {ld(a.inj_tab[j], i), ld(a.inj_tab[j + 1], i), ld(a.inj_tab[j + 2], i)};
+                static_assert(U::dot_fuses(3, 1, 1), "inj_delta and inj_tab normalised");
+                extra = U::add_n(extra, U::template dot_nr<3>(dl, tb));
+            } else if (left == 2) {
+                const U dl[2] = {cst(a.inj_delta[j]), cst(a.inj_delta[j + 1])}, tb[2] = {ld(a.inj_tab[j], i), ld(a.inj_tab[j + 1], i)};
+                extra = U::add_n(extra, U::template dot_nr<2>(dl, tb));
+            } else {
+                extra = U::add_n(extra, U::mul_nr(cst(a.inj_delta[j]), ld(a.inj_tab[j], i)));
+            }
+        }
+        const U qlm = U::add_n(ld(a.ql, i), U::mul_nr(ld(a.qm, i), r));
+        const U ga[3] = {qlm, ld(a.qr, i), ld(a.qo, i)}, gb[3] = {l, r, o};
+        static_assert(U::dot_fuses(3, 1, 1), "every operand normalised (add_n and mul_nr sweep)");
+        const U gate = U::add_n(extra, U::template dot_nr<3>(ga, gb));
         const U gm = cst(a.gamma), beta = cst(a.beta);
         const U lg = U::add_n(l, gm), rg = U::add_n(r, gm), og = U::add_n(o, gm);
         const U x = ld(a.x, i);
@@ -312,12 +347,13 @@
         U pb = U::mul_nr(z, U::add_n(lg, U::mul_nr(beta, x)));
         pb = U::mul_nr(pb, U::add_n(rg, U::mul_nr(cst(a.beta_u), x)));
         pb = U::mul_nr(pb, U::add_n(og, U::mul_nr(cst(a.beta_u2), x)));
-        const U perm = U::mul_nr(cst(a.alpha), U::template sub_k<2>(pa, pb));
         const Fr one_r = Fr::one();
         const U one = U::unpack(one_r.l);
-        const U loc = U::mul_nr(cst(a.alpha2), U::mul_nr(ld(a.l0, i), U::template sub_k<1>(z, one)));
-        const U num = U::add_n(U::add_n(gate, perm), loc);
-        const U res = U::template canon<1>(U::mul_nr(cst(a.zh_inv[i & 3]), num));
+        const U pc[2] = {cst(a.alpha), cst(a.alpha2)};
+        const U pv[2] = {U::template sub_k<2>(pa, pb), U::mul_nr(ld(a.l0, i), U::template sub_k<1>(z, one))};
+        static_assert(U::dot_fuses(2, 1, 1), "sub_k and mul_nr sweep");
+        const U num = U::add_n(gate, U::template dot_nr<2>(pc, pv));
+        const U res = U::template canon<1>(U::mul_nr(U::unpack(a.zh_inv[i & 3].l), num));
         Fr w;
         res.pack(w.l);
         out[jj] = w;
@@ -381,15 +417,24 @@
         __shared__ Fr sm[POLY_THREADS];
         const int p = blockIdx.y;
         const uint32_t t = threadIdx.x;
-        const Fr* f = a.f[p];
-        const Fr* __restrict__ pwp = a.pw[p] ? a.pw[p] : pw;
-        const uint32_t len = a.len[p];
+        const Fr* f = wave_uniform(a.f[p]);
+        const Fr* __restrict__ pwp = wave_uniform(a.pw[p] ? a.pw[p] : pw);
+        const uint32_t len = wave_uniform(a.len[p]);
         using U = FeU<FR>;
-        static_assert(U::HEADROOM >= 64 && EVAL_PER_THREAD * 2 <= 16, "8 products below 2 r each");
+        static_assert(U::HEADROOM >= 64 && EVAL_PER_THREAD % 2 == 0 && EVAL_PER_THREAD <= 16, "4 pairs below 2 r each");
+        static_assert(U::dot_fuses(2, 1, 1), "unpacked operands are normalised");
         U accu = U::zero();
-        for (int k = 0; k < EVAL_PER_THREAD; k++) {
-            uint32_t i = blockIdx.x * EVAL_BLOCK + k * POLY_THREADS + t;
-            if (i < len) { Fr a0 = f[i], b0 = pwp[i]; accu = U::add_n(accu, U::mul_nr(U::unpack(a0.l), U::unpack(b0.l))); }
+        for (int k = 0; k < EVAL_PER_THREAD; k += 2) {
+            const uint32_t i0 = blockIdx.x * EVAL_BLOCK + k * POLY_THREADS + t, i1 = i0 + POLY_THREADS;
+            if (i0 >= len) break;
+            Fr a0 = f[i0], b0 = pwp[i0];
+            if (i1 < len) {
+                Fr a1 = f[i1], b1 = pwp[i1];
+                const U fa[2] = {U::unpack(a0.l), U::unpack(a1.l)}, fb[2] = {U::unpack(b0.l), U::unpack(b1.l)};
+                accu = U::add_n(accu, U::template dot_nr<2>(fa, fb));
+            } else {
+                accu = U::add_n(accu, U::mul_nr(U::unpack(a0.l), U::unpack(b0.l)));
+            }
         }
         Fr acc;
         U::template canon<1>(U::template reduce_2p<8>(accu)).pack(acc.l);
@@ -456,6 +501,7 @@
 __global__ void __launch_bounds__(POLY_THREADS) derive_powers_kernel(DerivePowers<FR> a, const Fe<FR>* __restrict__ twu, uint32_t n, uint32_t count) { DerivePowersK<FR>::run(a, twu, n, count); }
 
 constexpr int LC_MAX = 20;
+constexpr int LC_GROUP = 6;
 template <class FR>
 struct LinCombArgs {
     const Fe<FR>* f[LC_MAX];
@@ -472,11 +518,22 @@
         using Fr = Fe<FR>;
         using U = FeU<FR>;
         static_assert(U::HEADROOM >= 64 && LC_MAX * 2 <= 64, "the sum of LC_MAX products below 2 r each must stay below 64 r");
+        static_assert(U::dot_fuses(LC_GROUP, 1, 1) && 2 * LC_GROUP <= 64, "coefficients and unpacked values are normalised (1, 1)");
         uint32_t i = blockIdx.x * blockDim.x + threadIdx.x;
         if (i >= a.out_len) return;
         U acc = U::zero();
-        for (int k = 0; k < a.count; k++)
-            if (i < a.len[k]) { Fr v = a.f[k][i]; acc = U::add_n(acc, U::mul_nr(U::unpack(a.coef[k].l), U::unpack(v.l))); }
+        for (int k = 0; k < a.count; k += LC_GROUP) {
+            const int end = k + LC_GROUP < a.count ? k + LC_GROUP : a.count;
+            typename U::Cols s = U::cols_zero();
+#pragma unroll 1
+            for (int t = k; t < end; t++) {
+                const Fr* __restrict__ ft = wave_uniform(a.f[t]);
+                const U c = U::unpack(wave_uniform(a.coef[t]).l);
+                __builtin_amdgcn_sched_barrier(0);
+                if (i < wave_uniform(a.len[t])) { Fr v = ft[i]; U::cols_mac(s, c, U::unpack(v.l)); }
+            }
+            acc = U::add_n(acc, U::template cols_reduce<LC_GROUP>(s));
+        }
         const U res = U::template canon<1>(U::template reduce_2p<32>(acc));
         Fr w;
         res.pack(w.l);
diff --git a/algoplonk_amd/csrc/selftest_ops.h b/algoplonk_amd/csrc/selftest_ops.h
--- a/algoplonk_amd/csrc/selftest_ops.h
+++ b/algoplonk_amd/csrc/selftest_ops.h
@@ -108,6 +108,30 @@
                 r.l[2] = U::sqr_takes(a.l[0]) ? 1u : 0u;
                 r.l[3] = (uint32_t)U::COLUMN_ROOM;
                 break;
+            case 50: case 51: case 52: case 53: {
+                const U x[7] = {a, c, a, c, a, b, a}, y[7] = {b, d, d, b, c, d, a};
+                r = op == 50 ? U::template dot_nr<1>(x, y) : op == 51 ? U::template dot_nr<2>(x, y)
+                  : op == 52 ? U::template dot_nr<3>(x, y) : U::template dot_nr<7>(x, y);
+                break;
+            }
+            case 54:
+                r.l[0] = U::dot_takes(a.l[0], a.l[1], a.l[2]) ? 1u : 0u;
+                r.l[1] = U::dot_fuses(a.l[0], a.l[1], a.l[2]) ? 1u : 0u;
+                break;
+            case 55: case 56: case 57: case 58: {
+                const U x[7] = {a, c, a, c, a, c, a}, y[7] = {b, d, d, b, b, d, d};
+                r = op == 55 ? U::template dot_nr<1, U::dot_max_factor(1)>(x, y) : op == 56 ? U::template dot_nr<2, U::dot_max_factor(2)>(x, y)
+                  : op == 57 ? U::template dot_nr<3, U::dot_max_factor(3)>(x, y) : U::template dot_nr<7, U::dot_max_factor(7)>(x, y);
+                break;
+            }
+            case 59: case 60: case 61: case 62: {
+                const U x[6] = {a, c, a, c, a, b}, y[6] = {b, d, d, b, c, d};
+                const int terms = op == 62 ? 6 : op - 58;
+                typename U::Cols s = U::cols_zero();
+                for (int t = 0; t < terms; t++) U::cols_mac(s, x[t], y[t]);
+                r = U::template cols_reduce<6>(s);
+                break;
+            }
             default: return SELFTEST_UNKNOWN_OP;
         }
         for (int i = 0; i < L; i++) out[i] = r.l[i];
diff --git a/algoplonk_amd/plonk.py b/algoplonk_amd/plonk.py
--- a/algoplonk_amd/plonk.py
+++ b/algoplonk_amd/plonk.py
@@ -108,7 +108,12 @@
     def paths(self, reset: bool = False) -> dict:
         pc = _lib.PathCounts()
         check(lib.apk_paths_read(self.ctx, C.byref(pc), int(reset)))
-        return pc.as_dict()
+        out = pc.as_dict()
+        if hasattr(lib, "apk_paths_read_more"):
+            more = _lib.PathCountsMore()
+            check(lib.apk_paths_read_more(self.ctx, C.byref(more), int(reset)))
+            out.update(more.as_dict())
+        return out
 
 
 @dataclass
diff --git a/include/apk.h b/include/apk.h
--- a/include/apk.h
+++ b/include/apk.h
@@ -356,6 +356,11 @@
     uint64_t msm_inplace;
 } apk_path_counts;
 int apk_paths_read(apk_ctx* ctx, apk_path_counts* out, int reset);
+typedef struct {
+    uint64_t coset_deferred;
+    uint64_t reserved[7];
+} apk_path_counts_more;
+int apk_paths_read_more(apk_ctx* ctx, apk_path_counts_more* out, int reset);
 
 typedef struct {
     uint32_t contexts;
```
